# sedaprotocol/bn254

Measured on AMD Instinct MI355X. Metric: BN254 pairings/sec (batch verify), higher is better.
Workload: dtype u32

## Files before the change

### bn254_amd/_native.py

```python
import ctypes
import os
import subprocess

_PKG = os.path.dirname(os.path.abspath(__file__))
_CSRC = os.path.join(_PKG, "csrc")
LIB_PATH = os.environ.get("BN254_LIB", os.path.join(_PKG, "libbn254hip.so"))
import glob


def translation_units():
    return sorted(glob.glob(os.path.join(_CSRC, "*.hip")))


def _dependencies():
    return translation_units() + sorted(glob.glob(os.path.join(_CSRC, "*.h"))) + sorted(glob.glob(os.path.join(_CSRC, "*.inc"))) + [
        os.path.join(_CSRC, "gen_constants.py"), os.path.join(_CSRC, "gen_step_asm.py"), os.path.join(os.path.dirname(_PKG), "include", "bn254_hip.h")]

HIPCC_COMPILE_FLAGS = ["-O3", "--offload-arch=gfx950", "-std=c++17", "-fPIC", "-mllvm", "-amdgpu-sched-strategy=max-ilp"]
HIPCC_LINK_FLAGS = ["--offload-arch=gfx950", "-shared", "-fPIC", "-Wl,--no-undefined"]
HIPCC_FLAGS = HIPCC_COMPILE_FLAGS + ["-shared", "-Wl,--no-undefined"]
_OBJ = os.path.join(_PKG, "build")


def _stale():
# ... 42 lines not shown
            print("libbn254hip.so: %d translation units compiled and linked in %.1f s" % (len(units), time.time() - t0), flush=True)
    return LIB_PATH


_lib = None


def load():
    global _lib
    if _lib is not None:
        return _lib
    if not os.path.exists(LIB_PATH):
        raise RuntimeError("libbn254hip.so is not built (run `python -c 'import __graft_entry__ as g; g.build()'`); "
                           "bn254_amd has no CPU fallback")
    L = ctypes.CDLL(LIB_PATH)
    vp, sz, u32, i32 = ctypes.c_void_p, ctypes.c_size_t, ctypes.c_uint32, ctypes.c_int
    L.bn254_version.restype = ctypes.c_char_p
    L.bn254_ctx_create.argtypes = [i32, ctypes.POINTER(vp)]
    L.bn254_ctx_destroy.argtypes = [vp]
    L.bn254_ctx_destroy.restype = None
    L.bn254_ctx_reserve.argtypes = [vp, sz]
    L.bn254_ctx_reserve_host.argtypes = [vp, sz, sz]
    L.bn254_ctx_synchronize.argtypes = [vp]
    L.bn254_ctx_set_profiling.argtypes = [vp, i32]
    L.bn254_ctx_expect_msgs_len.argtypes = [vp, ctypes.c_uint64]
    L.bn254_ctx_last_kernel_ms.argtypes = [vp, ctypes.POINTER(ctypes.c_float)]
    L.bn254_ctx_set_option.argtypes = [vp, i32, i32]
    L.bn254_debug_route_table.argtypes = [vp, ctypes.POINTER(ctypes.c_uint64), ctypes.POINTER(i32), ctypes.POINTER(i32), i32]
    L.bn254_debug_key_dedup_last.argtypes = [vp, ctypes.POINTER(ctypes.c_uint32)]
    if hasattr(L, "bn254_debug_key_cache_last"):
        L.bn254_debug_key_cache_last.argtypes = [vp, ctypes.POINTER(ctypes.c_uint32)]
    if hasattr(L, "bn254_debug_key_tables"):
        L.bn254_debug_key_tables.argtypes = [vp, i32, sz, sz, vp, vp, vp, vp]
    if hasattr(L, "bn254_debug_agg_tables"):
        L.bn254_debug_agg_tables.argtypes = [vp, i32, sz, sz, vp, vp]
    L.bn254_debug_agg_rand_last.argtypes = [vp, ctypes.POINTER(ctypes.c_uint64)]
    L.bn254_debug_agg_rand_sums.argtypes = [vp, ctypes.POINTER(ctypes.c_uint64), sz, sz, vp, vp, vp, vp, vp, vp]
    L.bn254_ctx_last_clocks.argtypes = [vp, ctypes.POINTER(ctypes.c_double)]
    L.bn254_batch_verify.argtypes = [vp, vp, vp, vp, vp, sz, u32, vp]
    L.bn254_batch_verify_device.argtypes = [vp, vp, vp, vp, vp, sz, u32, vp, vp]
    L.bn254_ctx_register_keys.argtypes = [vp, vp, sz, u32, vp]
    L.bn254_batch_verify_keyed.argtypes = [vp, vp, vp, vp, vp, sz, u32, vp]
    L.bn254_batch_verify_keyed_device.argtypes = [vp, vp, vp, vp, vp, sz, u32, vp, vp]
    L.bn254_batch_verify_keyed_bitmap.argtypes = [vp, vp, vp, vp, vp, sz, sz, u32, vp]
    L.bn254_batch_verify_keyed_bitmap_device.argtypes = [vp, vp, vp, vp, vp, sz, sz, u32, vp, vp]
    L.bn254_batch_verify_keyed_bitmap_randomized.argtypes = [vp, vp, vp, vp, vp, sz, sz, u32, vp, vp]
    L.bn254_batch_verify_keyed_bitmap_randomized_device.argtypes = [vp, vp, vp, vp, vp, sz, sz, u32, vp, vp, vp]
    L.bn254_batch_collect_keyed_bitmap.argtypes = [vp, vp, vp, vp, vp, vp, sz, sz, sz, u32, vp, vp, vp, vp, vp]
    L.bn254_batch_collect_keyed_bitmap_device.argtypes = [vp, vp, vp, vp, vp, vp, sz, sz, sz, u32, vp, vp, vp, vp, vp, vp]
    if hasattr(L, "bn254_batch_collect_keyed_bitmap_randomized"):
        L.bn254_batch_collect_keyed_bitmap_randomized.argtypes = [vp, vp, vp, vp, vp, vp, sz, sz, sz, u32, vp, vp, vp, vp, vp, vp]
        L.bn254_batch_collect_keyed_bitmap_randomized_device.argtypes = [vp, vp, vp, vp, vp, vp, sz, sz, sz, u32, vp, vp, vp, vp, vp, vp, vp]
        L.bn254_debug_collect_rand_last.argtypes = [vp, ctypes.POINTER(ctypes.c_uint64)]
    if hasattr(L, "bn254_batch_collect_keyed_bitmap_optimistic"):
        L.bn254_batch_collect_keyed_bitmap_optimistic.argtypes = [vp, vp, vp, vp, vp, vp, sz, sz, sz, u32, vp, vp, vp, vp, vp]
        L.bn254_batch_collect_keyed_bitmap_optimistic_device.argtypes = [vp, vp, vp, vp, vp, vp, sz, sz, sz, u32, vp, vp, vp, vp, vp, vp]
        L.bn254_debug_collect_opt_last.argtypes = [vp, ctypes.POINTER(ctypes.c_uint64)]
    if hasattr(L, "bn254_batch_merge_keyed_bitmap"):
        L.bn254_batch_merge_keyed_bitmap.argtypes = [vp, vp, vp, vp, vp, vp, sz, sz, sz, u32, vp, vp, vp, vp, vp, vp]
        L.bn254_batch_merge_keyed_bitmap_device.argtypes = [vp, vp, vp, vp, vp, vp, sz, sz, sz, u32, vp, vp, vp, vp, vp, vp, vp]
    L.bn254_debug_bitmap_rand_last.argtypes = [vp, ctypes.POINTER(ctypes.c_uint64)]
    L.bn254_debug_bitmap_rand_sums.argtypes = [vp, ctypes.POINTER(ctypes.c_uint64), sz, sz, vp, vp, vp, vp, vp, vp]
    L.bn254_batch_verify_keyed_randomized.argtypes = [vp, vp, vp, vp, vp, sz, u32, vp, vp]
    L.bn254_batch_verify_keyed_randomized_device.argtypes = [vp, vp, vp, vp, vp, sz, u32, vp, vp, vp]
    L.bn254_batch_verify_compressed.argtypes = [vp, vp, vp, vp, vp, sz, vp]
    L.bn254_batch_verify_compressed_device.argtypes = [vp, vp, vp, vp, vp, sz, vp, vp]
# ... 45 lines not shown
    L.bn254_mgpu_ctx.argtypes = [vp, i32]
    L.bn254_mgpu_ctx.restype = vp
    L.bn254_mgpu_shard_len.argtypes = [vp, sz]
    L.bn254_mgpu_shard_len.restype = sz
    L.bn254_mgpu_gathered_len.argtypes = [vp, sz]
    L.bn254_mgpu_gathered_len.restype = sz
    L.bn254_mgpu_shard_range.argtypes = [vp, sz, i32, ctypes.POINTER(sz), ctypes.POINTER(sz)]
    L.bn254_mgpu_reserve.argtypes = [vp, sz, i32]
    L.bn254_mgpu_synchronize.argtypes = [vp]
    L.bn254_mgpu_set_option.argtypes = [vp, i32, i32]
    L.bn254_mgpu_last_timing.argtypes = [vp, ctypes.POINTER(ctypes.c_float), ctypes.POINTER(ctypes.c_float)]
    L.bn254_mgpu_last_error.argtypes = [vp]
    L.bn254_mgpu_last_error.restype = ctypes.c_char_p
    L.bn254_mgpu_batch_verify.argtypes = [vp, vp, vp, vp, vp, sz, u32, vp]
    L.bn254_mgpu_batch_verify_device.argtypes = [vp, pp, pp, pp, pp, sz, u32, pp, pp]
    L.bn254_mgpu_batch_pairing.argtypes = [vp, vp, vp, sz, sz, u32, vp, vp, ctypes.POINTER(ctypes.c_uint64)]
    L.bn254_mgpu_batch_pairing_device.argtypes = [vp, pp, pp, sz, sz, u32, pp, pp, pp, pp]
    L.bn254_mgpu_batch_hash_to_g1.argtypes = [vp, vp, vp, sz, vp, vp, vp]
    L.bn254_mgpu_batch_verify_compressed.argtypes = [vp, vp, vp, vp, vp, sz, vp]
    L.bn254_mgpu_register_keys.argtypes = [vp, vp, sz, u32, vp]
    L.bn254_mgpu_batch_verify_keyed.argtypes = [vp, vp, vp, vp, vp, sz, u32, vp]
    L.bn254_mgpu_batch_aggregate_verify.argtypes = [vp, vp, vp, sz, vp, sz, vp, vp, vp, vp, sz, u32, vp]
    _lib = L
    return L


EXPORTED_SYMBOLS = [
    "bn254_version", "bn254_ctx_create", "bn254_ctx_destroy", "bn254_ctx_reserve", "bn254_ctx_reserve_host", "bn254_ctx_synchronize",
    "bn254_batch_verify", "bn254_batch_verify_device", "bn254_batch_verify_randomized", "bn254_batch_verify_randomized_device", "bn254_batch_verify_compressed", "bn254_batch_verify_compressed_device", "bn254_batch_hash_to_g1", "bn254_batch_hash_to_g1_device",
    "bn254_batch_pairing_check", "bn254_batch_pairing", "bn254_batch_pairing_device", "bn254_batch_check_public_keys",
    "bn254_batch_g1_add", "bn254_batch_g2_add", "bn254_batch_g1_mul", "bn254_batch_g2_mul", "bn254_batch_g1_mul_device",
    "bn254_batch_g2_mul_device", "bn254_batch_sign", "bn254_batch_sign_device", "bn254_batch_g1_sum", "bn254_batch_g2_sum",
    "bn254_batch_aggregate_verify", "bn254_batch_aggregate_verify_device", "bn254_ctx_register_pools", "bn254_ctx_register_pools_device",
    "bn254_batch_aggregate_verify_registered", "bn254_batch_aggregate_verify_registered_device", "bn254_batch_aggregate_verify_distinct", "bn254_batch_aggregate_verify_distinct_device", "bn254_batch_aggregate_verify_distinct_keyed", "bn254_batch_aggregate_verify_distinct_keyed_device", "bn254_batch_aggregate_verify_distinct_keyed_randomized", "bn254_batch_aggregate_verify_distinct_keyed_randomized_device", "bn254_batch_g1_decompress", "bn254_batch_g2_decompress", "bn254_debug_fp_op", "bn254_debug_fp12_op", "bn254_debug_final_exp_limbs", "bn254_debug_miller_loop", "bn254_debug_hash_candidate", "bn254_debug_route_table", "bn254_debug_key_dedup_last", "bn254_debug_key_cache_last", "bn254_debug_key_tables", "bn254_debug_agg_tables", "bn254_debug_agg_rand_last", "bn254_debug_agg_rand_sums", "bn254_probe_issue_rate", "bn254_probe_leaf_floor", "bn254_probe_fe_program", "bn254_ctx_set_profiling", "bn254_ctx_last_kernel_ms", "bn254_ctx_set_option", "bn254_ctx_last_clocks", "bn254_ctx_expect_msgs_len", "bn254_ctx_register_keys", "bn254_batch_verify_keyed", "bn254_batch_verify_keyed_device", "bn254_batch_verify_keyed_randomized", "bn254_batch_verify_keyed_randomized_device",
    "bn254_batch_verify_keyed_bitmap", "bn254_batch_verify_keyed_bitmap_device",
    "bn254_batch_verify_keyed_bitmap_randomized", "bn254_batch_verify_keyed_bitmap_randomized_device", "bn254_debug_bitmap_rand_last",
    "bn254_debug_bitmap_rand_sums", "bn254_batch_collect_keyed_bitmap", "bn254_batch_collect_keyed_bitmap_device",
    "bn254_batch_collect_keyed_bitmap_randomized", "bn254_batch_collect_keyed_bitmap_randomized_device", "bn254_debug_collect_rand_last",
    "bn254_batch_collect_keyed_bitmap_optimistic", "bn254_batch_collect_keyed_bitmap_optimistic_device", "bn254_debug_collect_opt_last",
    "bn254_batch_merge_keyed_bitmap", "bn254_batch_merge_keyed_bitmap_device",
    "bn254_mgpu_create", "bn254_mgpu_destroy", "bn254_mgpu_device_count", "bn254_mgpu_ctx", "bn254_mgpu_shard_len", "bn254_mgpu_shard_range",
    "bn254_mgpu_gathered_len", "bn254_mgpu_reserve", "bn254_mgpu_synchronize", "bn254_mgpu_set_option", "bn254_mgpu_last_timing",
    "bn254_mgpu_last_error", "bn254_mgpu_batch_verify", "bn254_mgpu_batch_verify_device", "bn254_mgpu_batch_pairing",
    "bn254_mgpu_batch_pairing_device", "bn254_mgpu_batch_hash_to_g1", "bn254_mgpu_batch_verify_compressed", "bn254_mgpu_register_keys",
    "bn254_mgpu_batch_verify_keyed", "bn254_mgpu_batch_aggregate_verify",
]
```

### bn254_amd/csrc/bn254_constants.h

```cpp
#pragma once

#define BN_LIMBS 9
#define BN_W 29
#define BN_MASK 0x1fffffffu
#define BN_HALF 0x10000000
#define BN_QL0 (-126026425)
#define BN_QL1 (17064119)
#define BN_QL2 (-59595953)
#define BN_QL3 (47522513)
#define BN_QL4 (-175777416)
#define BN_QL5 (47923393)
#define BN_QL6 (10936641)
#define BN_QL7 (240920116)
#define BN_QL8 (3171406)
#define BN_QL_ARRAY {BN_QL0, BN_QL1, BN_QL2, BN_QL3, BN_QL4, BN_QL5, BN_QL6, BN_QL7, BN_QL8}
#define BN_N0 0x4866389u
#define BN_TOP_PER_Q 3171406.4
#define BN_R_OVER_Q 169.285
#define BN_WEAK_KMUL 1354
#define BN_WEAK_HALF 1585703
#define BN_U_LO 0x4a6909f1u
#define BN_U_HI 0x44e992b4u
#define BN_N_FIXED_LINES 87

// ... 113 lines not shown
  {{{-200040337, -190665345, 184206374, 76585773, -122040462, 116307427, -3182763, -106971873, 150657}, {-124740882, -48385428, 25363536, -142741679, -158151770, -201941964, -78046412, -104889391, 1502077}}, {{262442771, 34913701, 54788380, -126213246, -261387237, 68871501, -237077543, 122771512, 3009073}, {201181020, -53518767, -160881225, 100319164, 169076449, -54190966, 48482503, 213128087, 857567}}, {{-176370655, -199481511, -128831276, 21759002, 178483129, -45989682, -237679608, 86689705, 903222}, {0, 0, 0, 0, 0, 0, 0, 0, 0}}},
  {{{-199390454, 140322044, -264541497, 218098246, 211463767, 115454738, 123055153, 108741638, 2871680}, {262069691, -87186243, -83201912, 117623600, -30263542, -203954648, 19394695, -190244704, 2253537}}, {{74861434, -57720419, -179314670, -230520040, 65997000, 207431631, 205002456, -66037731, 2120652}, {34392117, -71782572, -264376129, -127196325, 119748025, 203429416, -243176573, -113087350, 1664920}}, {{-176370655, -199481511, -128831276, 21759002, 178483129, -45989682, -237679608, 86689705, 903222}, {0, 0, 0, 0, 0, 0, 0, 0, 0}}},
  {{{-125164594, 203672984, 222121632, -236210239, 29018012, -120395034, -105765485, 146672474, 1819322}, {217134077, -112473868, -13365101, -155118944, 14561761, -163245527, 98054292, -116710799, 1869640}}, {{258779297, 86695130, -41789464, -146609841, -261957730, 146697339, -188270445, 166495143, 27148}, {190558376, -141717460, -92318918, -42801125, 160814942, -243365450, -98538843, 239515481, 2742811}}, {{-176370655, -199481511, -128831276, 21759002, 178483129, -45989682, -237679608, 86689705, 903222}, {0, 0, 0, 0, 0, 0, 0, 0, 0}}},
  {{{-266112787, -5731679, 64851336, 252971724, -4606107, -229625860, -38737421, 232289728, 1646670}, {139400236, -113999012, -78811786, -72939401, 136410247, 92762089, 170592144, 218767022, 1187664}}, {{-148581673, 144737950, -64941939, 266123669, -15806871, -65940181, -120563210, 222667854, 2161520}, {-157986495, 112576346, 175145252, 267211436, -125135784, -183314329, -112175291, -91287041, 2540137}}, {{-176370655, -199481511, -128831276, 21759002, 178483129, -45989682, -237679608, 86689705, 903222}, {0, 0, 0, 0, 0, 0, 0, 0, 0}}},
  {{{179936888, -35473748, -59679566, -5596775, -61480713, 10590727, 16868031, -259608724, 72786}, {176495202, -18815897, -120127598, 178871128, -200921685, 65070547, -58447813, 50527024, 2345596}}, {{208607304, 77283041, -66022222, 42098986, 268119722, 47691154, -142171534, -7679194, 862289}, {124395984, 158373343, -174933619, 134304166, 22689770, 39927471, -178412217, 229699851, 1515716}}, {{-176370655, -199481511, -128831276, 21759002, 178483129, -45989682, -237679608, 86689705, 903222}, {0, 0, 0, 0, 0, 0, 0, 0, 0}}},
  {{{-71531813, 67246960, 237949059, -177971974, -34822371, -224146645, -240850655, -104280605, 2152250}, {-128492592, 30948534, -112506348, 144871973, -7367378, -189697698, -93809008, 62946165, 301481}}, {{159384783, 221847505, -90488723, 22146507, 211531190, 7432841, 132374126, 114003879, 2065160}, {-241377406, 181464060, 7646761, -26472298, -241841179, 120193515, -8498110, -73364135, 1809262}}, {{-176370655, -199481511, -128831276, 21759002, 178483129, -45989682, -237679608, 86689705, 903222}, {0, 0, 0, 0, 0, 0, 0, 0, 0}}},
  {{{-171428400, -249458482, -70035234, 152428224, 268237382, -178271449, 27520838, -120671971, 3068723}, {9932335, -197646614, 142498572, 83337858, -109958741, -179274817, -15833319, -69914058, 96617}}, {{94843765, -103780142, 157119612, -56869585, 15912524, -34614887, 195919263, 64907236, 920143}, {118941173, -98073096, -136818613, 244594129, 129041635, -41694611, 139884983, -259883868, 2705119}}, {{-176370655, -199481511, -128831276, 21759002, 178483129, -45989682, -237679608, 86689705, 903222}, {0, 0, 0, 0, 0, 0, 0, 0, 0}}},
  {{{243121283, -245146285, -156305461, -12818002, -178365131, -177158676, -256937671, 34668348, 75137}, {10333938, -37755957, 72278169, 85086581, 92939512, -72886985, -38751985, -227509480, 925099}}, {{-147192708, 258120271, -41162607, 42078054, -163913536, -119625961, -44844893, 185883765, 1188799}, {235579323, 193778380, -13294417, 159229682, 236601368, 192779425, 13781851, 93907330, 933591}}, {{-176370655, -199481511, -128831276, 21759002, 178483129, -45989682, -237679608, 86689705, 903222}, {0, 0, 0, 0, 0, 0, 0, 0, 0}}},
  {{{-141907892, -107977127, 204683730, 3373323, 96002441, 139722946, -95095458, 134243936, 1812559}, {-185199286, 263934561, 257143555, -179990218, -145893234, -224382509, 102131607, -29198656, 2532873}}, {{-58711793, 245191909, 92638325, 90256483, -67674438, 231377561, -260854161, 176023936, 1608472}, {4908704, -73766975, -173992501, -266421877, -120394349, 39964257, 175000575, 265420786, 33071}}, {{-176370655, -199481511, -128831276, 21759002, 178483129, -45989682, -237679608, 86689705, 903222}, {0, 0, 0, 0, 0, 0, 0, 0, 0}}},
  {{{-214306326, 112995705, 203217010, -45483838, -252784442, 120321467, 186528369, -146789637, 162579}, {-156386064, 217762605, 78321876, 140823106, 185638832, -1785707, -231401731, -203083753, 1261828}}, {{106508173, -117204588, 216647907, 7709844, 200022610, 227507439, 80806348, -181739761, 2784693}, {9540569, -27897884, 155658076, -57119890, -242306310, 11065481, -1829803, -22755391, 2526826}}, {{-176370655, -199481511, -128831276, 21759002, 178483129, -45989682, -237679608, 86689705, 903222}, {0, 0, 0, 0, 0, 0, 0, 0, 0}}},
  {{{-170550275, -131985597, 141986177, 263500420, 33397427, 74369277, 162661307, 152195668, 2661521}, {-81853459, 202864132, 22294944, 1719661, -95127053, -45787432, 169589203, -103112267, 1178675}}, {{-174079808, -51588416, -57795799, 247696906, 234371116, 81952568, 176965714, 50459872, 931029}, {237866458, -125584815, 256714432, 155783857, 144310399, 78795867, 220130107, 123179926, 166919}}, {{-176370655, -199481511, -128831276, 21759002, 178483129, -45989682, -237679608, 86689705, 903222}, {0, 0, 0, 0, 0, 0, 0, 0, 0}}},
  {{{-49306564, -92009915, 76714808, 206425296, -18911896, -89494543, -107789449, 141625555, 1865807}, {234514699, 122766930, -104413407, 106700060, 155636159, 205375446, -46091338, 255081650, 1234052}}, {{-212032201, -36621430, -150832888, -35484420, 162963214, 74033470, -189370026, 17664498, 1423930}, {-163470212, 81285382, -38833882, 108922757, -50181724, -225338663, 149676106, -228450571, 1376109}}, {{-176370655, -199481511, -128831276, 21759002, 178483129, -45989682, -237679608, 86689705, 903222}, {0, 0, 0, 0, 0, 0, 0, 0, 0}}},
  {{{-229545731, -249242282, 48482127, 32812434, -18338362, 126217735, 118954546, 26723153, 3004994}, {-10570593, -188510812, -217780881, -107498616, -165303242, 167964699, -36064246, 75691970, 1723376}}, {{15185324, -47571680, 127749242, -157459636, -41466509, 118054769, -207995470, 153028387, 1037592}, {-39021391, 70955764, 142262821, -130870691, -68729247, -236203824, 80363762, -77152138, 2702413}}, {{-176370655, -199481511, -128831276, 21759002, 178483129, -45989682, -237679608, 86689705, 903222}, {0, 0, 0, 0, 0, 0, 0, 0, 0}}},
  {{{163647724, 192924703, -162630789, -118076012, 142975318, 168169548, -89538170, 62909519, 2094264}, {-214163828, -230767358, -189956325, -157148179, -247498553, -255153517, -236790193, -34715494, 1715569}}, {{115587364, 258688938, -51849393, 78842177, -262068265, -107185610, -221650625, 193176103, 2588549}, {-75559992, 259688436, -77911971, 263346331, 190183004, -143954193, 130301912, -208291216, 317805}}, {{-176370655, -199481511, -128831276, 21759002, 178483129, -45989682, -237679608, 86689705, 903222}, {0, 0, 0, 0, 0, 0, 0, 0, 0}}},
  {{{-21443416, 248752699, 24211503, 180647149, -11004787, -169352692, 24828521, 208236708, 731906}, {240734963, -945267, -94409694, 224890492, -222082203, 95326662, 93146178, -163322462, 3124303}}, {{101170552, 13205284, -256511354, -18535751, -226284632, -14711015, -169989660, 215698512, 1214444}, {-115335139, -243410446, 167591371, 70040109, -111466827, -44550076, 42921127, -61055270, 936229}}, {{-176370655, -199481511, -128831276, 21759002, 178483129, -45989682, -237679608, 86689705, 903222}, {0, 0, 0, 0, 0, 0, 0, 0, 0}}},
  {{{194475413, 66556270, 33163353, 214495719, 84714233, -151129526, 158231720, -178379680, 1711252}, {-23886822, -68860429, -104616143, 50480129, -8681874, 206104951, -153610971, 202107973, 321501}}, {{-265102970, -155790835, 234719479, -118893583, 56555457, 176278835, 16057839, 193352116, 2911462}, {-214060094, -226278758, 210925259, -256654959, -206288843, 143191197, 216026142, -121889172, 2063704}}, {{-176370655, -199481511, -128831276, 21759002, 178483129, -45989682, -237679608, 86689705, 903222}, {0, 0, 0, 0, 0, 0, 0, 0, 0}}},
  {{{211995304, -114933848, -204710941, -153849488, 137386204, -57436494, -268383413, -176836654, 1163802}, {-119692606, -106057472, 24474457, -121620700, -140419497, 254002587, 237930320, 29624771, 1466741}}, {{-33408981, 77861381, -12995667, -26474951, 14983613, -156197272, -230468610, -7322544, 1255074}, {-100843488, 117663684, 224808907, -230128445, -198040350, 198331391, 234252901, 187672035, 1495249}}, {{-176370655, -199481511, -128831276, 21759002, 178483129, -45989682, -237679608, 86689705, 903222}, {0, 0, 0, 0, 0, 0, 0, 0, 0}}},
  {{{258650570, -35612775, -200285181, -53517004, -198078314, 147873122, -124934989, -14800304, 448573}, {198251006, 96238494, -178994434, 246685808, 193583880, -169066857, 132738305, 46917062, 1657838}}, {{-242372727, 175863385, -63652076, 251445205, -120227698, -230194405, -137499659, -69733145, 2549436}, {244579158, -9827117, -175975206, -190679677, -59209720, 68734345, -233140879, -236722399, 958296}}, {{-176370655, -199481511, -128831276, 21759002, 178483129, -45989682, -237679608, 86689705, 903222}, {0, 0, 0, 0, 0, 0, 0, 0, 0}}},
  {{{-118181686, 191380492, 46891918, -67496608, 133499266, 136775164, -30652145, -159719896, 141374}, {111447810, 81254940, 236294220, 176317818, -51431853, 4048663, 76515630, -194841446, 1230674}}, {{-57107160, 30848795, 86177915, 178230363, 173484625, 111107460, -139935602, -160260691, 2613107}, {-14902460, -53830383, -70833480, 265851823, -125813216, -209271761, 172380324, -61621536, 3082156}}, {{-176370655, -199481511, -128831276, 21759002, 178483129, -45989682, -237679608, 86689705, 903222}, {0, 0, 0, 0, 0, 0, 0, 0, 0}}},
  {{{184814613, 51899031, 233603478, 258659516, 153972936, 23890032, -133142987, -88543576, 1729823}, {192270751, -8658243, 214299070, 149087285, 211026243, -164366848, 251037918, -66480647, 1848146}}, {{211883601, 54930164, 101866637, -237060239, -36819856, -9497778, 174962490, 257398535, 482184}, {18982256, -123882900, 239342450, 21201073, -221501387, 220773893, -39037341, -267961371, 1577083}}, {{-176370655, -199481511, -128831276, 21759002, 178483129, -45989682, -237679608, 86689705, 903222}, {0, 0, 0, 0, 0, 0, 0, 0, 0}}},
  {{{-133312880, 263585465, 16353286, 194981750, 46178582, 115018734, -167817870, 139318092, 2068671}, {102282468, 148314672, -30682414, 199717073, -239073256, -242076110, -263081100, 42274790, 1894594}}, {{-105249443, 58595139, 13996760, -101554426, -4112982, 178467927, -44373279, 120348143, 1755967}, {114840994, -148286844, 180095703, -2116349, 92320787, 224277985, 155350517, -133487757, 749870}}, {{-176370655, -199481511, -128831276, 21759002, 178483129, -45989682, -237679608, 86689705, 903222}, {0, 0, 0, 0, 0, 0, 0, 0, 0}}},
  {{{-48534465, -216407913, -80449945, 197826411, 28844792, -79138690, -244010556, 186112668, 655732}, {-135627737, -219576662, -43600977, 162482618, 166965224, -181199647, 124866808, 75750459, 1878572}}, {{-74728592, -13595521, -87696240, -51211358, 144286912, 201058004, 12627411, -252447748, 2293052}, {31278092, -87291687, 250215026, 250101657, -122853210, 185162931, 115541449, -237945290, 2101663}}, {{-176370655, -199481511, -128831276, 21759002, 178483129, -45989682, -237679608, 86689705, 903222}, {0, 0, 0, 0, 0, 0, 0, 0, 0}}},
  {{{1920732, -177274209, -94106247, -259622463, 198105170, -77279384, 152108594, 207918834, 273777}, {-137525945, 121461598, -13360930, 249712992, 198210032, 30308474, -77309931, -199784788, 734443}}, {{263023313, -259909195, -178730994, -171277393, -50243763, -207558859, 132438671, -254036575, 2614219}, {2299910, -80464943, 249430672, 178951382, 4286762, 184744822, 154232506, 259713016, 120390}}, {{-176370655, -199481511, -128831276, 21759002, 178483129, -45989682, -237679608, 86689705, 903222}, {0, 0, 0, 0, 0, 0, 0, 0, 0}}},
  {{{-166807573, 257561474, 5758311, 16562045, 154704719, -115989712, 30296549, 212095792, 2382072}, {-214218106, 109893984, 260431646, 253247344, 185804414, 147228457, -149769418, -248037657, 2745144}}, {{254155362, -31231806, -262802243, 127284760, 189343100, -188982993, 50947556, 54876934, 753175}, {-181976431, -56200449, -228230263, 261245934, -133178743, 254970581, 132113466, -232840218, 2676942}}, {{-176370655, -199481511, -128831276, 21759002, 178483129, -45989682, -237679608, 86689705, 903222}, {0, 0, 0, 0, 0, 0, 0, 0, 0}}},
  {{{37112481, 129068714, 2231463, 118245711, 73714168, 14136474, -227005073, 114158147, 1452017}, {-241524548, -219338631, -195709013, -49076846, -61142324, 95780292, -127092311, -233650515, 105673}}, {{42977708, -76007726, 195561301, -171725564, -264048364, 121600305, -211248172, 30495361, 460408}, {216640771, -129426574, -148041264, -106105658, 8450471, 125953370, -107989583, 70858773, 2231587}}, {{-176370655, -199481511, -128831276, 21759002, 178483129, -45989682, -237679608, 86689705, 903222}, {0, 0, 0, 0, 0, 0, 0, 0, 0}}},
  {{{-3232440, -230912943, -165435285, -161296496, 181300732, -186576993, 158514743, -102527308, 178806}, {213156407, -97026260, 105562298, -60297714, -35770377, -231575633, 106944355, 130250462, 2063018}}, {{-265998852, 226199746, 182911214, -64753753, 196257397, -115603873, 257355951, -248162796, 1250972}, {-43343060, -31181880, -185052752, 87259796, -169372165, -102536487, 194779497, -263472281, 973169}}, {{-176370655, -199481511, -128831276, 21759002, 178483129, -45989682, -237679608, 86689705, 903222}, {0, 0, 0, 0, 0, 0, 0, 0, 0}}},
  {{{88056784, -7863797, 2393509, 189566777, -4124281, 43222830, 74388923, 115793747, 1596681}, {-61490741, 166590202, -262009048, -241222290, 151032788, 152243465, -198708223, 133601828, 1001776}}, {{170428225, 28120576, 158580597, -267158179, -205070664, -193272982, -118866539, 48154750, 763669}, {-87919621, 83255079, -89948094, 44678235, 224783456, 153742904, 120397335, -139364349, 1815208}}, {{-176370655, -199481511, -128831276, 21759002, 178483129, -45989682, -237679608, 86689705, 903222}, {0, 0, 0, 0, 0, 0, 0, 0, 0}}},
  {{{262805377, 25131819, -207131569, -169166008, -77129595, -74240946, -108282114, -244472810, 517945}, {-93130162, -94355081, 64587666, 84777866, -90920406, -8820760, 139744111, 142454513, 1344638}}, {{84178301, -101967244, -185592134, 124907746, 8864191, -181416434, 175900991, 37214613, 2250176}, {-71996750, -249770878, 32060657, 100694729, -248824792, 157385725, -54255296, -114993530, 1691525}}, {{-176370655, -199481511, -128831276, 21759002, 178483129, -45989682, -237679608, 86689705, 903222}, {0, 0, 0, 0, 0, 0, 0, 0, 0}}},
  {{{4468045, -257270474, -212501869, -201875648, 247931930, -69039740, -10866934, -159837900, 418727}, {-195131113, -26854457, -113740685, -179567795, 87499462, -64426147, -249940327, 257223239, 2328593}}, {{127008600, 119343077, 52409536, -7940586, 111211957, 54407389, -42873706, 203151225, 3108489}, {231539509, -140691144, -164724047, -33026607, 26982684, -156904521, 265339498, -46944075, 2243270}}, {{-176370655, -199481511, -128831276, 21759002, 178483129, -45989682, -237679608, 86689705, 903222}, {0, 0, 0, 0, 0, 0, 0, 0, 0}}},
  {{{-44891955, 90630318, -67087730, 24812910, 95403380, 185541070, 22421094, -48123712, 1870376}, {-114359724, 212759385, -155669803, -13087971, 118129017, -193674558, -98888558, 197073061, 793579}}, {{89208724, -233383300, -79197354, -1132594, -265691887, 247209455, -245705599, -187369324, 99477}, {206283919, -105467383, -216114661, 73440443, -137125806, -220635920, -73680286, 25048480, 941390}}, {{-176370655, -199481511, -128831276, 21759002, 178483129, -45989682, -237679608, 86689705, 903222}, {0, 0, 0, 0, 0, 0, 0, 0, 0}}},
  {{{-162397500, 2954997, 152488182, -65669248, -2226221, 126434462, 136504248, -45920178, 1018187}, {37038594, -230220348, -39757353, 51278743, 94503435, 69559177, 117383119, -38335104, 1747986}}, {{-168849216, 266245294, 103631925, -116049438, -183139901, -68554844, 259384813, -968803, 1609363}, {215323032, -48099119, -244987994, -57467655, -73007447, -145862608, -75994125, -187878897, 359235}}, {{-176370655, -199481511, -128831276, 21759002, 178483129, -45989682, -237679608, 86689705, 903222}, {0, 0, 0, 0, 0, 0, 0, 0, 0}}},
  {{{198924502, -95920802, 109010388, 97989720, -212428967, 216061620, -144460110, 93801757, 1223757}, {-249735650, 57427941, 134749786, -254932027, 35573088, 90419683, 133149999, 143547148, 125881}}, {{194882581, 87312206, -43835174, -161184211, 204737166, -171525322, -265395304, 139734743, 2318771}, {-210600565, -38893026, 17554950, -242192057, 58146045, -142126381, 157173323, 44273995, 2017346}}, {{-176370655, -199481511, -128831276, 21759002, 178483129, -45989682, -237679608, 86689705, 903222}, {0, 0, 0, 0, 0, 0, 0, 0, 0}}},
};
```

### bn254_amd/csrc/bn254_devhooks.hip

```cpp
#include <hip/hip_runtime.h>

#include <cstdio>
#include <cstdlib>
#include <cstring>
#include <new>

#include "../../include/bn254_hip.h"
#include "bn254_hash.h"
#include "bn254_io.h"
#include "bn254_pairing.h"

using namespace bn254;

#include "bn254_ws.h"
#include "bn254_lane.h"
#include "bn254_host.h"

KERNEL_SMALL void k_debug_fp_op(int op, const uint8_t* a, const uint8_t* b, size_t n, uint8_t* out, uint8_t* status) {
  size_t i = (size_t)blockIdx.x * BN_WAVE + threadIdx.x;
  if (i >= n) return;
  uint32_t any = 0;
  Fp x, y, r;
  bool ok = fp_from_be(x, a + 32 * i, any);
  if (b) ok = fp_from_be(y, b + 32 * i, any) && ok; else y = fp_zero();
// ... 192 lines not shown
    if (!c->kd_last_run || !c->kd_ctl || !c->kd_lines_last) return BN254_E_BAD_ARGUMENT;
    HIP_TRY(hipMemcpy(ctl, c->kd_ctl, sizeof ctl, hipMemcpyDeviceToHost));
    if (first + count > ctl[KD_CTL_D] || first + count > c->kd_keys_cap) return BN254_E_BAD_ARGUMENT;
    if (ctl[KD_CTL_BUILD] + ctl[KD_CTL_HITS] != ctl[KD_CTL_D]) return BN254_E_BAD_ARGUMENT;
    if (rep) HIP_TRY(hipMemcpy(rep, c->kd_rep_last + first, count * sizeof(uint32_t), hipMemcpyDeviceToHost));
    const size_t cap = c->kd_keys_cap;
    uint8_t* h = (uint8_t*)malloc(count * sizeof(uint32_t) + 2 * cap + 1);
    if (!h) return BN254_E_NO_MEMORY;
    const uint32_t* rows = (const uint32_t*)h;
    uint8_t *h_st = h + count * sizeof(uint32_t), *h_inf = h_st + cap;
    hipError_t e = count ? hipMemcpy(h, c->kd_row_of_last + first, count * sizeof(uint32_t), hipMemcpyDeviceToHost) : hipSuccess;
    if (e == hipSuccess) e = hipMemcpy(h_st, c->kd_st_last, cap, hipMemcpyDeviceToHost);
    if (e == hipSuccess) e = hipMemcpy(h_inf, c->kd_inf_last, cap, hipMemcpyDeviceToHost);
    int rc = e == hipSuccess ? 0 : -(int)e;
    for (size_t k = 0; k < count && !rc; ++k) {
      const size_t r = rows[k];
      if (r >= cap) { rc = BN254_E_BAD_ARGUMENT; break; }
      e = hipMemcpy(lines + k * per_key, c->kd_lines_last + r * per_key, per_key * sizeof(int32_t), hipMemcpyDeviceToHost);
      if (e != hipSuccess) rc = -(int)e;
      if (st) st[k] = h_st[r];
      if (inf) inf[k] = h_inf[r];
    }
    free(h);
    return rc;
  } else {
    if (!c->key_lines || first + count > c->n_keys) return BN254_E_BAD_ARGUMENT;
    src = c->key_lines; src_st = c->key_st; src_inf = c->key_inf;
  }
  HIP_TRY(hipMemcpy(lines, src + first * per_key, count * per_key * sizeof(int32_t), hipMemcpyDeviceToHost));
  if (st) HIP_TRY(hipMemcpy(st, src_st + first, count, hipMemcpyDeviceToHost));
  if (inf) HIP_TRY(hipMemcpy(inf, src_inf + first, count, hipMemcpyDeviceToHost));
  return 0;
}
static int debug_rand_last(bn254_ctx* c, int ran, const uint32_t* stats, uint64_t out[6]) {
  if (!c || !out) return BN254_E_BAD_ARGUMENT;
  for (int i = 0; i < 6; ++i) out[i] = 0;
  if (!ran || !stats) return 0;
  HIP_TRY(hipSetDevice(c->device));
  HIP_TRY(hipDeviceSynchronize());
  uint32_t st[5];
  HIP_TRY(hipMemcpy(st, stats, sizeof st, hipMemcpyDeviceToHost));
  out[0] = 1;
  for (int i = 0; i < 5; ++i) out[i + 1] = st[i];
  return 0;
}
int bn254_debug_agg_rand_last(bn254_ctx* c, uint64_t out[6]) { return debug_rand_last(c, c ? c->aggr_last_ran : 0, c ? c->aggr_stats : nullptr, out); }
int bn254_debug_bitmap_rand_last(bn254_ctx* c, uint64_t out[6]) { return debug_rand_last(c, c ? c->bmr_last_ran : 0, c ? c->bmr_stats : nullptr, out); }
int bn254_debug_collect_rand_last(bn254_ctx* c, uint64_t out[4]) {
  if (!c || !out) return BN254_E_BAD_ARGUMENT;
  for (int i = 0; i < 4; ++i) out[i] = 0;
  if (!c->clr_last_ran || !c->clr_stats) return 0;
  HIP_TRY(hipSetDevice(c->device));
  HIP_TRY(hipDeviceSynchronize());
  uint32_t st[4];
  HIP_TRY(hipMemcpy(st, c->clr_stats, sizeof st, hipMemcpyDeviceToHost));
  for (int i = 0; i < 4; ++i) out[i] = st[i];
  return 0;
}
int bn254_debug_collect_opt_last(bn254_ctx* c, uint64_t out[4]) {
  if (!c || !out) return BN254_E_BAD_ARGUMENT;
  for (int i = 0; i < 4; ++i) out[i] = 0;
  if (!c->clo_last_ran || !c->clo_stats) return 0;
  HIP_TRY(hipSetDevice(c->device));
  HIP_TRY(hipDeviceSynchronize());
  uint32_t st[4];
  HIP_TRY(hipMemcpy(st, c->clo_stats, sizeof st, hipMemcpyDeviceToHost));
// ... 206 lines not shown
```

### bn254_amd/csrc/bn254_hip.hip

```cpp
#include <hip/hip_runtime.h>
#include <thread>

#include <cstdio>
#include <cstdlib>
#include <cstring>
#include <new>

#include "../../include/bn254_hip.h"
#include "bn254_hash.h"
#include "bn254_io.h"
#include "bn254_pairing.h"

using namespace bn254;

#include "bn254_ws.h"
#include "bn254_lane.h"
#include "bn254_host.h"

KERNEL_SMALL void k_decode_g1(const uint8_t* pts, size_t n, uint32_t flags, Ws ws, int px, int inf_plane, int accumulate) {
  size_t i = (size_t)blockIdx.x * BN_WAVE + threadIdx.x;
  if (i >= n) return;
  G1Affine p;
  uint8_t st = decode_g1(p, pts + 64 * i, flags);
  if (st != ST_OK) g1_set_generator(p);
// ... 392 lines not shown
  if (c->max_chunk > 0) return n > (size_t)c->max_chunk ? (size_t)c->max_chunk : 0;
  if (n * ws_per_item <= c->ws.stride && (!key_dedup || (n <= c->kd_items_cap && (size_t)c->kd_max_keys <= c->kd_keys_cap))) return 0;
  const size_t per_item = ws_per_item * WS_BYTES_PER_ITEM + (key_dedup ? KD_BYTES_PER_ITEM : 0);
  const size_t fixed = key_dedup ? (size_t)c->kd_max_keys * KD_BYTES_PER_KEY : 0;
  size_t avail;
  if (c->assume_free_mb > 0) avail = (size_t)c->assume_free_mb << 20;
  else {
    size_t fr = 0, total = 0;
    if (hipSetDevice(c->device) != hipSuccess || hipMemGetInfo(&fr, &total) != hipSuccess) { (void)hipGetLastError(); return 0; }
    avail = fr + c->ws.stride * WS_BYTES_PER_ITEM + c->kd_items_cap * KD_BYTES_PER_ITEM + c->kd_keys_cap * KD_BYTES_PER_KEY;
  }
  const size_t need = ((n + 255) & ~(size_t)255) * per_item + fixed;
  if (need <= avail / 10 * 9) return 0;
  const size_t room = avail / 10 * 8 > fixed ? avail / 10 * 8 - fixed : 0;
  size_t chunk = room / per_item;
  chunk &= ~(size_t)65535;
  if (chunk == 0) chunk = room / per_item & ~(size_t)255;
  if (key_dedup && (chunk == 0 || route_for(c, chunk).miller != BN_ML_LANE_PAIRS)) return ws_chunk_for(c, n, ws_per_item, false);
  return chunk && chunk < n ? chunk : 0;
}
#define KD_NO_ROOM 1
static int kd_reserve(bn254_ctx* c, size_t n, KeyDedup& kd) {
  size_t slots = 1;
  while (slots < 2 * n) slots <<= 1;
  const size_t keys = (size_t)c->kd_max_keys;
  if (n > c->kd_items_cap || keys > c->kd_keys_cap) {
    const size_t items_cap = n > c->kd_items_cap ? ((n + 255) & ~(size_t)255) : c->kd_items_cap;
    const size_t keys_cap = keys > c->kd_keys_cap ? keys : c->kd_keys_cap;
    { int rc_ = ctx_quiesce(c); if (rc_) return rc_; }
    if (c->kd_buf) { HIP_TRY(hipFree(c->kd_buf)); c->kd_buf = nullptr; }
    c->kd_items_cap = c->kd_keys_cap = 0;
    c->kd_ctl = nullptr;
    c->kd_lines_last = nullptr;
    c->kd_cache_valid = false;
    if (hipMalloc((void**)&c->kd_buf, items_cap * KD_BYTES_PER_ITEM + keys_cap * KD_BYTES_PER_KEY + 512) != hipSuccess) {
      (void)hipGetLastError();
      c->kd_buf = nullptr;
      return KD_NO_ROOM;
    }
    c->kd_items_cap = items_cap;
    c->kd_keys_cap = keys_cap;
  }
  size_t slots_cap = 1;
  while (slots_cap < 2 * c->kd_items_cap) slots_cap <<= 1;
  uint8_t* p = c->kd_buf;
  auto take = [&](size_t bytes) { uint8_t* r = p; p += (bytes + 15) & ~(size_t)15; return r; };
  kd.table = (uint32_t*)take(slots_cap * 4);
  kd.slot_id = (uint32_t*)take(slots_cap * 4);
  kd.slot_of = (uint32_t*)take(c->kd_items_cap * 4);
  kd.key_idx = (uint32_t*)take(c->kd_items_cap * 4);
  kd.lines = (int32_t*)take(c->kd_keys_cap * BN_N_FIXED_LINES * BN_KEY_LINE_WORDS * 4);
  kd.c2 = (int32_t*)take(c->kd_keys_cap * BN_N_FIXED_LINES * 2 * BN_LIMBS * 4);
  kd.rep = (uint32_t*)take(c->kd_keys_cap * 4);
  kd.ctl = (uint32_t*)take(KD_CTL_WORDS * 4);
  c->kd_ctl = kd.ctl;
  kd.st = take(c->kd_keys_cap);
  kd.inf = take(c->kd_keys_cap);
  kd.row_of = (uint32_t*)take(c->kd_keys_cap * 4);
  kd.build_row = (uint32_t*)take(c->kd_keys_cap * 4);
  kd.build_rep = (uint32_t*)take(c->kd_keys_cap * 4);
  kd.c_keys = (uint32_t*)take(c->kd_keys_cap * 128);
  size_t index_slots = 1;
  while (index_slots < 2 * keys) index_slots <<= 1;
  kd.c_index = (uint32_t*)take(4 * c->kd_keys_cap * 4);
  kd.c_state = (uint32_t*)take(4);
  kd.index_mask = (uint32_t)(index_slots - 1);
  c->kd_lines_last = kd.lines; c->kd_rep_last = kd.rep; c->kd_st_last = kd.st; c->kd_inf_last = kd.inf; c->kd_row_of_last = kd.row_of;
  kd.slot_mask = (uint32_t)(slots - 1);
  kd.hash_mask = c->kd_hash_bits > 0 && c->kd_hash_bits < 32 ? (1u << c->kd_hash_bits) - 1 : 0xFFFFFFFFu;
  kd.max_keys = (uint32_t)keys;
  kd.min_mult = (uint32_t)c->kd_min_mult;
  return 0;
}
int scratch_reserve(bn254_ctx* c, uint8_t** buf, size_t* cap, size_t bytes) {
  if (bytes <= *cap) return 0;
  { int rc_ = ctx_quiesce(c); if (rc_) return rc_; }
  if (*buf) { HIP_TRY(hipFree(*buf)); *buf = nullptr; *cap = 0; }
  const size_t grown = (bytes + 4095) & ~(size_t)4095;
  HIP_TRY(hipMalloc((void**)buf, grown));
  *cap = grown;
  return 0;
}
int stage_reserve(bn254_ctx* c, int slot, size_t bytes) {
  if (bytes <= c->stage_cap[slot]) return 0;
  HIP_TRY(hipSetDevice(c->device));
  return scratch_reserve(c, &c->stage[slot], &c->stage_cap[slot], bytes);
}
uint8_t* HostStaging::out(int slot, size_t bytes, void* host) {
  if (!rc) rc = stage_reserve(c, slot, bytes);
  if (rc) return nullptr;
  if (host) copy_back(host, c->stage[slot], bytes);
  return c->stage[slot];
}
uint8_t* HostStaging::in(int slot, const void* host, size_t bytes) {
  uint8_t* d = out(slot, bytes ? bytes : 1);
  if (d && bytes) check(hipMemcpyAsync(d, host, bytes, hipMemcpyHostToDevice, c->stream));
  return rc ? nullptr : d;
}
void HostStaging::copy_back(void* host, const void* dev, size_t bytes) {
  if (!host || !bytes) return;
// ... 170 lines not shown
  c->pair_lanes = 1;
  c->rand_min_batch = RAND_MIN_BATCH_DEFAULT;
  c->agg_rand_min_pairs = AGG_RAND_MIN_PAIRS_DEFAULT;
  c->agg_rand_group_pairs = AGG_RAND_GROUP_PAIRS_DEFAULT;
  c->bmr_min_tuples = BITMAP_RAND_MIN_TUPLES_DEFAULT;
  c->bmr_group_tuples = BITMAP_RAND_GROUP_TUPLES_DEFAULT;
  c->bmr_max_keys = BITMAP_RAND_MAX_KEYS_DEFAULT;
  c->collect_wave_min = COLLECT_WAVE_MIN_SHARES_DEFAULT;
  c->collect_rand_min_shares = COLLECT_RAND_MIN_SHARES_DEFAULT;
  c->collect_rand_min_per_key = COLLECT_RAND_MIN_PER_KEY_DEFAULT;
  c->collect_opt_min_shares = COLLECT_OPT_MIN_SHARES_DEFAULT;
  c->collect_opt_min_tuple_shares = COLLECT_OPT_MIN_TUPLE_SHARES_DEFAULT;
  c->merge_wave_min = MERGE_WAVE_MIN_PARTS_DEFAULT;
  c->trio_max_batch = TRIO_MAX_BATCH_DEFAULT;
  c->hash_direct_width = HASH_DIRECT_WIDTH_DEFAULT;
  c->hash_tail_chunk = HASH_TAIL_CHUNK_DEFAULT;
  c->trio_wave_roles = TRIO_WAVE_ROLES_DEFAULT;
  c->agg_subset_min_tuples = AGG_SUBSET_MIN_TUPLES_DEFAULT;
  c->agg_sort_by_msg = 1;
  c->agg_t4_route = 0;
  c->agg_wide_min_tuples = AGG_WIDE_MIN_TUPLES_DEFAULT;
  c->pinned_staging = PINNED_STAGING_DEFAULT;
  c->fits_w8 = bn254_quad_fits_device(1); c->fits_quad = bn254_quad_fits_device(0); c->fits_trio = bn254_trio_fits_device();
  if (c->trio_wave_roles == 2 && !c->fits_w8) c->trio_wave_roles = 1;
  if (c->trio_wave_roles == 1 && !c->fits_quad) c->trio_wave_roles = 0;
  if (!c->fits_trio) c->trio_max_batch = 0;
  c->nonet_max_batch = bn254_nonet_fits_device() ? NONET_MAX_BATCH_DEFAULT : 0;
  c->lm_max_batch = bn254_lm_fits_device() ? LM_MAX_BATCH_DEFAULT : 0;
  c->nonet_wide = 1;
  c->g2_fixed_base = 1;
  c->key_dedup = 1;
  c->kd_max_keys = KEY_DEDUP_MAX_KEYS_DEFAULT;
  c->kd_min_mult = KEY_DEDUP_MIN_MULT_DEFAULT;
  c->kd_cache = 1;
  c->bm_table_max_keys = BITMAP_TABLE_MAX_KEYS_DEFAULT;
  c->device = hip_device;
  hipError_t err = hipStreamCreateWithFlags(&c->stream, hipStreamNonBlocking);
  if (err == hipSuccess) err = hipStreamCreateWithFlags(&c->copy_stream, hipStreamNonBlocking);
  if (err == hipSuccess) err = hipEventCreateWithFlags(&c->copy_done, hipEventDisableTiming);
  if (err == hipSuccess) err = hipEventCreateWithFlags(&c->last_done, hipEventDisableTiming);
  if (err == hipSuccess) err = hipStreamCreateWithFlags(&c->kd_stream, hipStreamNonBlocking);
  if (err == hipSuccess) err = hipEventCreateWithFlags(&c->kd_fork, hipEventDisableTiming);
  if (err == hipSuccess) err = hipEventCreateWithFlags(&c->kd_join, hipEventDisableTiming);
  if (err == hipSuccess) err = hipEventCreateWithFlags(&c->kd_done, hipEventDisableTiming);
  for (int i = 0; i < 5 && err == hipSuccess; ++i) err = hipEventCreate(&c->ev[i]);
  if (err != hipSuccess) {
    if (c->kd_done) (void)hipEventDestroy(c->kd_done);
    if (c->kd_join) (void)hipEventDestroy(c->kd_join);
    if (c->kd_fork) (void)hipEventDestroy(c->kd_fork);
    if (c->kd_stream) (void)hipStreamDestroy(c->kd_stream);
    if (c->last_done) (void)hipEventDestroy(c->last_done);
    for (int i = 0; i < 5; ++i) if (c->ev[i]) (void)hipEventDestroy(c->ev[i]);
    if (c->copy_done) (void)hipEventDestroy(c->copy_done);
    if (c->copy_stream) (void)hipStreamDestroy(c->copy_stream);
    if (c->stream) (void)hipStreamDestroy(c->stream);
    delete c;
    return -(int)err;
  }
  *out = c;
  return 0;
}
void bn254_ctx_destroy(bn254_ctx* c) {
  if (!c) return;
  (void)hipSetDevice(c->device);
  (void)ctx_quiesce(c);
  if (c->ws.planes) (void)hipFree(c->ws.planes);
// ... 94 lines not shown
    c->nonet_max_batch = value;
    return 0;
  }
  if (option == BN254_OPT_NONET_WIDE) { c->nonet_wide = value != 0; return 0; }
  if (option == BN254_OPT_LM_MAX_BATCH) {
    HIP_TRY(hipSetDevice(c->device));
    if (value < 0 || (value > 0 && !bn254_lm_fits_device())) return BN254_E_BAD_ARGUMENT;
    c->lm_max_batch = value;
    return 0;
  }
  if (option == BN254_OPT_PINNED_STAGING) { if (value < 0 || value > 16) return BN254_E_BAD_ARGUMENT; c->pinned_staging = value; return 0; }
  if (option == BN254_OPT_AGG_SORT_BY_MSG) { c->agg_sort_by_msg = value != 0; return 0; }
  if (option == BN254_OPT_AGG_T4_ROUTE) { if (value < 0 || value > 1) return BN254_E_BAD_ARGUMENT; c->agg_t4_route = value; return 0; }
  if (option == BN254_OPT_AGG_WIDE_MIN_TUPLES) { if (value < 0) return BN254_E_BAD_ARGUMENT; c->agg_wide_min_tuples = value; return 0; }
  if (option == BN254_OPT_CLOCK_PROBE) {
    HIP_TRY(hipSetDevice(c->device));
    HIP_TRY(hipDeviceSynchronize());
    if (value && !c->ws.clk) {
      HIP_TRY(hipMalloc((void**)&c->ws.clk, sizeof(unsigned long long) * 3 * BN_CLK_MAX_WG * 2));
      HIP_TRY(hipMemset(c->ws.clk, 0, sizeof(unsigned long long) * 3 * BN_CLK_MAX_WG * 2));
    } else if (!value && c->ws.clk) {
      HIP_TRY(hipFree(c->ws.clk));
      c->ws.clk = nullptr;
    }
    return 0;
  }
  if (option == BN254_OPT_HASH_MAX_TRIES) { if (value < 0 || value > 255) return BN254_E_BAD_ARGUMENT; c->hash_max_tries = value; return 0; }
  if (option == BN254_OPT_G2_FIXED_BASE) { c->g2_fixed_base = value != 0; return 0; }
  if (option == BN254_OPT_MAX_CHUNK) { if (value < 0) return BN254_E_BAD_ARGUMENT; c->max_chunk = value; return 0; }
  if (option == BN254_OPT_ASSUME_FREE_MB) { if (value < 0) return BN254_E_BAD_ARGUMENT; c->assume_free_mb = value; return 0; }
  if (option == BN254_OPT_KEY_DEDUP) { if (value < 0 || value > 1) return BN254_E_BAD_ARGUMENT; c->key_dedup = value; return 0; }
  if (option == BN254_OPT_KEY_DEDUP_MAX_KEYS) { if (value < 0 || value > KEY_DEDUP_MAX_KEYS_LIMIT) return BN254_E_BAD_ARGUMENT; c->kd_max_keys = value; return 0; }
  if (option == BN254_OPT_KEY_DEDUP_MIN_MULT) { if (value < 1) return BN254_E_BAD_ARGUMENT; c->kd_min_mult = value; return 0; }
  if (option == BN254_OPT_KEY_DEDUP_FORCE_GENERIC) { c->kd_force_generic = value == 2 ? 2 : value != 0; return 0; }
  if (option == BN254_OPT_KEY_CACHE) { if (value < 0 || value > 1) return BN254_E_BAD_ARGUMENT; c->kd_cache = value; c->kd_cache_valid = false; return 0; }
  if (option == BN254_OPT_KEY_DEDUP_HASH_BITS) { if (value < 0 || value > 32) return BN254_E_BAD_ARGUMENT; c->kd_hash_bits = value; return 0; }
  if (option == BN254_OPT_AGGD_KEYED_ROUTE) { if (value < 0 || value > 3) return BN254_E_BAD_ARGUMENT; c->aggd_keyed_route = value; return 0; }
  if (option == BN254_OPT_AGG_RAND_MIN_PAIRS) { if (value < 0) return BN254_E_BAD_ARGUMENT; c->agg_rand_min_pairs = value; return 0; }
  if (option == BN254_OPT_AGG_RAND_GROUP_PAIRS) { if (value < 1) return BN254_E_BAD_ARGUMENT; c->agg_rand_group_pairs = value; return 0; }
  if (option == BN254_OPT_BITMAP_TABLE_MAX_KEYS) { if (value < 0) return BN254_E_BAD_ARGUMENT; c->bm_table_max_keys = value; return 0; }
  if (option == BN254_OPT_BITMAP_RAND_MIN_TUPLES) { if (value < 0) return BN254_E_BAD_ARGUMENT; c->bmr_min_tuples = value; return 0; }
  if (option == BN254_OPT_BITMAP_RAND_MAX_KEYS) { if (value < 0) return BN254_E_BAD_ARGUMENT; c->bmr_max_keys = value; return 0; }
  if (option == BN254_OPT_COLLECT_WAVE_MIN_SHARES) { if (value < 1) return BN254_E_BAD_ARGUMENT; c->collect_wave_min = value; return 0; }
  if (option == BN254_OPT_COLLECT_RAND_MIN_SHARES) { if (value < 0) return BN254_E_BAD_ARGUMENT; c->collect_rand_min_shares = value; return 0; }
  if (option == BN254_OPT_COLLECT_RAND_MIN_PER_KEY) { if (value < 0) return BN254_E_BAD_ARGUMENT; c->collect_rand_min_per_key = value; return 0; }
  if (option == BN254_OPT_COLLECT_OPT_MIN_SHARES) { if (value < 0) return BN254_E_BAD_ARGUMENT; c->collect_opt_min_shares = value; return 0; }
  if (option == BN254_OPT_MERGE_WAVE_MIN_PARTS) { if (value < 1) return BN254_E_BAD_ARGUMENT; c->merge_wave_min = value; return 0; }
  if (option == BN254_OPT_COLLECT_OPT_MIN_TUPLE_SHARES) { if (value < 0) return BN254_E_BAD_ARGUMENT; c->collect_opt_min_tuple_shares = value; return 0; }
  if (option == BN254_OPT_BITMAP_RAND_GROUP_TUPLES) { if (value < 1) return BN254_E_BAD_ARGUMENT; c->bmr_group_tuples = value; return 0; }
  if (option == BN254_OPT_BITMAP_ROUTE) { if (value < 0 || value > 2) return BN254_E_BAD_ARGUMENT; c->bm_route = value; return 0; }
  return BN254_E_BAD_ARGUMENT;
}
int bn254_ctx_last_clocks(bn254_ctx* c, double sclk_mhz[3]) {
  if (!c || !sclk_mhz || !c->ws.clk) return BN254_E_BAD_ARGUMENT;
  HIP_TRY(hipSetDevice(c->device));
  int wall_khz = 0;
  HIP_TRY(hipDeviceGetAttribute(&wall_khz, hipDeviceAttributeWallClockRate, c->device));
  const size_t words = (size_t)3 * BN_CLK_MAX_WG * 2;
  unsigned long long* h = (unsigned long long*)malloc(words * sizeof(unsigned long long));
  if (!h) return BN254_E_NO_MEMORY;
  hipError_t e = hipDeviceSynchronize();
  if (e == hipSuccess) e = hipMemcpy(h, c->ws.clk, words * sizeof(unsigned long long), hipMemcpyDeviceToHost);
  if (e == hipSuccess) e = hipMemset(c->ws.clk, 0, words * sizeof(unsigned long long));
  if (e != hipSuccess) { free(h); return -(int)e; }
  for (int k = 0; k < 3; ++k) {
    double cyc = 0, wall = 0;
// ... 30 lines not shown
    default: return bn254_pair_final_exp(n, c->ws, use_hash, d_status, nullptr, nullptr, s);
  }
}
int launch_verify_miller_fe(bn254_ctx* c, hipStream_t s, size_t n, int pairs, int use_hash, uint8_t* d_status, bool mark) {
  if (!c->pair_lanes) {
    const unsigned g = grid_for(n);
    if (pairs == BN_PAIRS_CHECK_PKS) k_miller_cpk<<<g, BN_WAVE, 0, s>>>(n, c->ws);
    else k_miller_verify<<<g, BN_WAVE, 0, s>>>(n, c->ws, nullptr, nullptr);
    if (mark) PROF_MARK(3);
    k_final_exp<<<g, BN_WAVE, 0, s>>>(n, 1, 1, 1, c->ws, use_hash, nullptr, d_status, 0, 0, nullptr, nullptr);
    return 0;
  }
  const BnRoute r = route_for(c, n);
  int rc;
  switch (r.miller) {
    case BN_ML_LANE_MACHINE: rc = bn254_lm_miller_verify(n, c->ws, s, pairs); break;
    case BN_ML_WAVE_ROLES:
      rc = c->trio_wave_roles == 2 ? bn254_w8_miller_verify(n, c->ws, s, pairs)
           : c->trio_wave_roles ? bn254_quad_miller_verify(n, c->ws, s, pairs) : bn254_trio_miller_verify(n, c->ws, s, pairs);
      break;
    default: rc = bn254_pair_miller_verify(n, c->ws, nullptr, nullptr, s, pairs); break;
  }
  if (rc) return rc;
  if (mark) PROF_MARK(3);
  return launch_final_exp_layout(c, s, n, use_hash, d_status, r.fe);
}

extern "C" {
static int verify_tail(bn254_ctx* c, hipStream_t s, size_t n, uint8_t* d_status, bool split, const KeyDedup* kd, int hash_first) {
  int rc;
  if (kd) {
    HIP_TRY(hipStreamWaitEvent(s, c->kd_join, 0));
    const KeyTable kt = {kd->lines, kd->st, kd->inf, kd->max_keys};
    if ((rc = bn254_pair_miller_verify_keyed(n, c->ws, kd->key_idx, kt, s, 0, nullptr, kd->ctl + KD_CTL_KEYED_N))) return rc;
    if ((rc = bn254_pair_miller_verify(n, c->ws, nullptr, kd->ctl + KD_CTL_GENERIC_N, s))) return rc;
    PROF_MARK(3);
    if ((rc = bn254_pair_final_exp(n, c->ws, 1, d_status, nullptr, nullptr, s))) return rc;
    HIP_TRY(hipEventRecord(c->kd_done, s));
  } else if (split) {
    const unsigned g = grid_for(n);
    k_miller_verify_split<<<2 * g, BN_WAVE, 0, s>>>(n, c->ws.stride / 2, g, c->ws);
    PROF_MARK(3);
    k_final_exp<<<g, BN_WAVE, 0, s>>>(n, 2, 1, c->ws.stride / 2, c->ws, 1, nullptr, d_status, 0, 0, nullptr, nullptr);
  } else if ((rc = launch_verify_miller_fe(c, s, n, BN_PAIRS_VERIFY, 1, d_status, true))) return rc;
  PROF_MARK(4);
  prof_done(c, hash_first ? EV_HASH_FIRST : EV_DECODE_FIRST);
  HIP_TRY(hipGetLastError());
  return 0;
}
static int verify_after_decode(bn254_ctx* c, hipStream_t s, const uint8_t* d_msgs, const uint64_t* d_off, size_t n, uint8_t* d_status, bool split,
                               const KeyDedup* kd = nullptr) {
  PROF_MARK(1);
  if (const int rc = launch_hash_rounds(c, s, d_msgs, d_off, n, PL_P2X, BY_P2_INF, nullptr)) return rc;
  PROF_MARK(2);
  return verify_tail(c, s, n, d_status, split, kd, 0);
}

int bn254_batch_verify_device(bn254_ctx* c, const uint8_t* d_msgs, const uint64_t* d_off, const uint8_t* d_sigs, const uint8_t* d_pks,
                              size_t n, uint32_t flags, uint8_t* d_status, void* stream) {
  MsgsLenScope msgs_len_scope(c);
  if (!c || (n && (!d_msgs || !d_off || !d_sigs || !d_pks || !d_status))) return BN254_E_BAD_ARGUMENT;
  if (n == 0) return 0;
  if (misaligned(d_sigs) || misaligned(d_pks) || ((uintptr_t)d_off & 7u)) return BN254_E_MISALIGNED;
  HIP_TRY(hipSetDevice(c->device));
  bool split = c->split_miller && n <= BN_SPLIT_MAX_N;
  bool key_dedup = c->key_dedup && c->kd_max_keys > 0 && c->pair_lanes && !split && n <= 0xFFFFFFFFu &&
                         route_for(c, n).miller == BN_ML_LANE_PAIRS && route_for(c, n).fe == BN_FE_LANE_PAIRS;
// ... 309 lines not shown
```

### bn254_amd/csrc/bn254_host.h

```cpp
#pragma once
#include <hip/hip_runtime.h>

#include <cstdint>
#include <cstdlib>
#include <cstring>
#include <new>

#include "../../include/bn254_hip.h"

#define BN_HIDDEN __attribute__((visibility("hidden")))

struct AggTables { int valid; size_t n_msgs, n_signers, n_groups, groups4, built_for; int wide2, wide1, t4_builder; };

struct AggrLast { size_t ng, cbase, tbase; const uint32_t *nagg, *bkey; const uint64_t *glo, *ghi; const uint8_t* gst; };

enum EvLayout { EV_DECODE_FIRST = 0, EV_HASH_FIRST = 1, EV_COLLECT = 2 };

struct bn254_ctx {
  int device;
  hipStream_t stream;
  Ws ws;
  uint8_t* stage[8];
  size_t stage_cap[8];
  int profiling;
// ... 21 lines not shown
  int ev_valid;
  int ev_layout;
  hipStream_t copy_stream;
  uint8_t* pin;
  size_t pin_cap;
  int pinned_staging;
  hipEvent_t copy_done;
  uint64_t msgs_len_next;
  int msgs_len_declared;
  uint64_t msgs_len_call;
  int entry_depth;
  int32_t* key_lines;
  int32_t* key_xy;
  uint8_t* key_st;
  uint8_t* key_inf;
  size_t n_keys, key_cap;
  hipEvent_t last_done;
  bool last_done_armed;
  Pool g2_comb;
  int g2_comb_ready;
  Pool g1_comb;
  int g1_comb_ready;
  int g2_fixed_base;
  AggTables reg_pools;
  int max_chunk;
  int assume_free_mb;
  bool fits_w8, fits_quad, fits_trio;
  uint8_t* aggd_buf;
  size_t aggd_cap;
  int key_dedup;
  int kd_max_keys;
  int kd_min_mult;
  int kd_force_generic;
  int kd_hash_bits;
  hipStream_t kd_stream;
  hipEvent_t kd_fork, kd_join;
  hipEvent_t kd_done;
  int kd_cache;
  bool kd_cache_valid;
  uint32_t kd_cache_flags;
  int kd_cache_max_keys, kd_cache_hash_bits;
  uint8_t* kd_buf;
  size_t kd_items_cap, kd_keys_cap;
  uint32_t* kd_ctl;
  const int32_t* kd_lines_last;
  const uint32_t* kd_rep_last;
  const uint32_t* kd_row_of_last;
  const uint8_t *kd_st_last, *kd_inf_last;
  int kd_last_run;
  int aggd_keyed_route;
  int agg_rand_min_pairs;
  int agg_rand_group_pairs;
  uint8_t* aggr_buf;
  size_t aggr_cap;
  uint32_t* aggr_stats;
  int aggr_last_ran;
  AggrLast aggr_last;
  uint8_t* bm_bad;
  size_t bm_bad_cap;
  uint8_t* bm_tab;
  size_t bm_tab_cap;
  bool bm_bad_valid, bm_tab_valid;
  int bm_table_max_keys;
  int bm_route;
  int bmr_min_tuples;
  int bmr_group_tuples;
  int bmr_max_keys;
  uint8_t* bmr_buf;
  size_t bmr_cap;
  uint32_t* bmr_stats;
  int bmr_last_ran;
  AggrLast bmr_last;
  uint8_t* collect_buf;
  size_t collect_cap;
  int collect_wave_min;
  int collect_rand_min_shares;
  int collect_rand_min_per_key;
  uint32_t* clr_stats;
// ... 150 lines not shown
```

### bn254_amd/csrc/bn254_keydedup.h

```cpp
#pragma once

namespace bn254 {

template <class Emit>
BN_DEV bool kd_walk_raw_lines(const G2Affine& q, Emit&& emit) {
  G2Proj t;
  LineCoef l;
  t.x = q.x; t.y = q.y; t.z = fp2_one();
  const Fp2 q_yneg = fp2_neg(q.y);
  bool degenerate = false;
  int idx = 0;
  auto line = [&]() {
    const Fp2 c2 = NR(290, l.c2);
    degenerate = fp2_is_zero(c2) || degenerate;
    emit(idx++, NS(292, l.c0), NS(293, l.c1), c2);
  };
#if defined(__HIPCC__)
#pragma clang loop unroll(disable)
#endif
  for (int d = 0; d < 64; ++d) {
    dbl_step(t, l); line();
    const int digit = C_ATE_NAF[d];
    if (digit != 0) { add_step(t, l, q.x, fp2_select(digit > 0, q.y, q_yneg)); line(); }
  }
  add_step(t, l, fp2_mul(fp2_conj(q.x), fp2_load_const(C_TW_FROB_X1)), fp2_mul(fp2_conj(q.y), fp2_load_const(C_TW_FROB_Y1))); line();
  add_step(t, l, fp2_mul(q.x, fp2_load_const(C_TW_FROB_X2)), q.y); line();
  return degenerate;
}
BN_DEV void kd_scale_line(const Fp2& c0, const Fp2& c1, const Fp2& c2, Fp2& r0, Fp2& r1) {
  const Fp2 inv = NS(291, fp2_inv(c2));
  const Fp2 a = fp2_mul(c0, inv), b = fp2_mul(c1, inv);
  BN_FOR_ROLES(k) { r0.c[k] = fp_canon(a.c[k]); r1.c[k] = fp_canon(b.c[k]); }
}

#define KD_TREE_LEAVES 128
#define KD_TREE_LEVELS 7
#if !defined(__HIPCC__)
static inline void kd_scale_tree(const Fp2* c0, const Fp2* c1, const Fp2* c2, Fp2* r0, Fp2* r1) {
  static_assert(BN_N_FIXED_LINES <= KD_TREE_LEAVES && (1 << KD_TREE_LEVELS) == KD_TREE_LEAVES, "tree shape");
  Fp2 prod[2 * KD_TREE_LEAVES], inv[2 * KD_TREE_LEAVES];
  for (int p = 0; p < KD_TREE_LEAVES; ++p) prod[KD_TREE_LEAVES + p] = p < BN_N_FIXED_LINES ? fp2_reduce_weak(c2[p]) : fp2_one();
  for (int w = KD_TREE_LEAVES / 2; w >= 1; w >>= 1)
    for (int node = w; node < 2 * w; ++node) prod[node] = fp2_mul(prod[2 * node], prod[2 * node + 1]);
  inv[1] = fp2_inv(prod[1]);
  for (int w = 2; w <= KD_TREE_LEAVES; w <<= 1)
    for (int node = w; node < 2 * w; ++node) inv[node] = fp2_mul(inv[node >> 1], prod[node ^ 1]);
  for (int p = 0; p < BN_N_FIXED_LINES; ++p) {
    const Fp2 a = fp2_mul(c0[p], inv[KD_TREE_LEAVES + p]), b = fp2_mul(c1[p], inv[KD_TREE_LEAVES + p]);
    BN_FOR_ROLES(k) { r0[p].c[k] = fp_canon(a.c[k]); r1[p].c[k] = fp_canon(b.c[k]); }
  }
}
#endif

#if defined(__HIPCC__)
BN_DEV bool load_fp_be_checked(Fp& r, const uint8_t* p, uint32_t& any) {
  const uint32_t* w = (const uint32_t*)p;
  U256 t;
#pragma unroll
  for (int k = 0; k < 8; ++k) { t.w[7 - k] = __builtin_bswap32(w[k]); any |= w[k]; }
  bool ok = !u256_geq(t.w, C_Q);
  r = fp_from_u256(t);
  return ok;
}
BN_DEV uint8_t decode_g2_pair_role(G2Affine& q, const uint8_t* b, uint32_t flags) {
  const unsigned role = threadIdx.x & 1u;
  uint32_t any = 0;
  bool ok = load_fp_be_checked(q.x.c[0], b + 32 * role, any);
  ok = load_fp_be_checked(q.y.c[0], b + 64 + 32 * role, any) && ok;
  any |= (uint32_t)bn_partner_word((int32_t)any);
  ok = bn_pair_and(ok);
  q.inf = any == 0;
  uint8_t st = ST_OK;
  if (q.inf) st = (flags & FLAG_REJECT_IDENTITY) ? (uint8_t)ST_INVALID_GROUP_POINT : (uint8_t)ST_OK;
  else if (!ok) st = ST_NOT_MEMBER;
  const bool on_curve = g2_on_curve(q);
  if (st == ST_OK && !q.inf && !on_curve) st = ST_INVALID_GROUP_POINT;
  return st;
}
#endif

}
```

### bn254_amd/csrc/bn254_keydedup.hip

```cpp
#include <hip/hip_runtime.h>

#define BN_SPLIT_FP2 1
#define bn254 bn254_kd
#include "bn254_pairing.h"
#include "bn254_keydedup.h"
#include "bn254_lmachine.h"
#include "bn254_kdlines.h"

using namespace bn254;

#include "bn254_ws.h"

#define KD_WG 256
#define KERNEL_KD_PAIR __global__ __launch_bounds__(KD_WG) __attribute__((amdgpu_waves_per_eu(2, 2)))
#define KERNEL_KD __global__ __launch_bounds__(KD_WG)

__device__ __forceinline__ uint32_t kd_hash(const uint32_t* w, uint32_t hash_mask) {
  uint32_t h = 0x9E3779B9u;
#pragma unroll
  for (int k = 0; k < 32; ++k) {
    h ^= w[k];
    h *= 0x85EBCA6Bu;
    h ^= h >> 13;
  }
// ... 185 lines not shown
    if (live && pair < 3) kd_store_own(c == 2 ? c2s + (size_t)idx * 2 * BN_LIMBS : rows + (size_t)idx * BN_KEY_LINE_WORDS + (size_t)c * 2 * BN_LIMBS, v);
  }
};
KERNEL_KD_LM void k_kd_lines(const uint8_t* pks, uint32_t flags, KeyDedup kd, int report_degenerate) {
  const uint32_t d = kd.ctl[KD_CTL_BUILD];
  if ((uint32_t)blockIdx.x * KD_LM_PER_WAVE >= d) return;
  __builtin_amdgcn_s_setprio(3);
  const unsigned l = threadIdx.x, v = l / KD_LM_LANES, role = l & 1u;
  KdLmDev m;
  m.writer = v < KD_LM_PER_WAVE;
  const unsigned vslot = m.writer ? v : KD_LM_PER_WAVE - 1;
  m.pair = (l % KD_LM_LANES) >> 1;
  uint32_t j = (uint32_t)blockIdx.x * KD_LM_PER_WAVE + vslot;
  m.live = m.writer && j < d;
  if (j >= d) j = d - 1;
  const uint32_t row = kd.build_row[j];
  m.bx.base = vslot * KD_LM_KEY_STRIDE + role * KD_LM_ROLE_STRIDE;
  G2Affine q;
  const uint8_t st = decode_g2_pair_role(q, pks + 128 * (size_t)kd.build_rep[j], flags);
  const bool real = st == ST_OK && !q.inf;
  if (!real) { q.x = fp2_load_const(C_G2_GEN[0]); q.y = fp2_load_const(C_G2_GEN[1]); }
  if (m.live && m.pair == 0 && role == 0) { kd.st[row] = st; kd.inf[row] = q.inf; }
  if (m.writer) {
    m.bx.put(m.bx.slot(LS_ZERO), fp2_zero()); m.bx.put(m.bx.slot(LS_DUMMY), fp2_zero());
    kd_builder_init(m.bx, q);
  }
#pragma unroll
  for (int lv = 0; lv < KD_LV_N; ++lv) {
    const LmEntry* t = kd_level_table(lv);
#pragma unroll
    for (int k = 0; k < 5; ++k) m.e[lv].w[k] = t[m.pair].w[k];
  }
  m.rows = kd.lines + (size_t)row * BN_N_FIXED_LINES * BN_KEY_LINE_WORDS;
  m.c2s = kd.c2 + (size_t)row * BN_N_FIXED_LINES * 2 * BN_LIMBS;
  m.degenerate = false;
  KD_LM_FENCE();
  kd_builder_program(m);
  if (m.live && ((real && m.degenerate) || report_degenerate) && m.pair == 0 && role == 0) atomicOr(&kd.ctl[KD_CTL_FLAGS], (uint32_t)KD_DEGENERATE);
}
static_assert(BN_N_FIXED_LINES <= KD_TREE_LEAVES && 2 * KD_TREE_LEAVES == KD_WG, "one lane pair per leaf");
#define KD_NODE_WORDS (2 * BN_LIMBS)
KERNEL_KD_PAIR void k_kd_scale(KeyDedup kd) {
  if (blockIdx.x >= kd.ctl[KD_CTL_BUILD]) return;
  const uint32_t j = kd.build_row[blockIdx.x];
  __shared__ int32_t prod[2 * KD_TREE_LEAVES * KD_NODE_WORDS];
  __shared__ int32_t inv[2 * KD_TREE_LEAVES * KD_NODE_WORDS];
  const uint32_t p = threadIdx.x >> 1;
  const bool line = p < BN_N_FIXED_LINES;
  int32_t* row = kd.lines + ((size_t)j * BN_N_FIXED_LINES + (line ? p : 0u)) * BN_KEY_LINE_WORDS;
  {
    Fp2 leaf = fp2_one();
    if (line) leaf = fp2_reduce_weak(kd_load_own(kd.c2 + ((size_t)j * BN_N_FIXED_LINES + p) * KD_NODE_WORDS));
    kd_store_own(prod + (KD_TREE_LEAVES + p) * KD_NODE_WORDS, leaf);
  }
  __syncthreads();
  for (uint32_t w = KD_TREE_LEAVES / 2; w >= 1; w >>= 1) {
    if (p < w) {
      const uint32_t node = w + p;
      kd_store_own(prod + node * KD_NODE_WORDS, fp2_mul(kd_load_own(prod + 2 * node * KD_NODE_WORDS), kd_load_own(prod + (2 * node + 1) * KD_NODE_WORDS)));
    }
    __syncthreads();
  }
  if (threadIdx.x < BN_WAVE) {
    const Fp2 r = fp2_inv(kd_load_own(prod + KD_NODE_WORDS));
    if (p == 0) kd_store_own(inv + KD_NODE_WORDS, r);
  }
  __syncthreads();
  for (uint32_t w = 2; w <= KD_TREE_LEAVES; w <<= 1) {
    if (p < w) {
      const uint32_t node = w + p;
      kd_store_own(inv + node * KD_NODE_WORDS, fp2_mul(kd_load_own(inv + (node >> 1) * KD_NODE_WORDS), kd_load_own(prod + (node ^ 1u) * KD_NODE_WORDS)));
    }
    __syncthreads();
  }
  if (!line) return;
  const Fp2 c2inv = kd_load_own(inv + (KD_TREE_LEAVES + p) * KD_NODE_WORDS);
  const Fp2 a = fp2_mul(kd_load_own(row), c2inv), b = fp2_mul(kd_load_own(row + 2 * BN_LIMBS), c2inv);
  Fp2 r0, r1;
  BN_FOR_ROLES(k) { r0.c[k] = fp_canon(a.c[k]); r1.c[k] = fp_canon(b.c[k]); }
  kd_store_own(row, r0);
  kd_store_own(row + 2 * BN_LIMBS, r1);
}
KERNEL_KD void k_kd_decide(size_t n, KeyDedup kd, int force_generic, int cache_on) {
  const bool keyed = force_generic != 1 && kd_viable(kd, n) && (kd.ctl[KD_CTL_FLAGS] & KD_DEGENERATE) == 0;
  if (threadIdx.x == 0) {
    kd.ctl[KD_CTL_KEYED_N] = keyed ? (uint32_t)n : 0u;
    kd.ctl[KD_CTL_GENERIC_N] = keyed ? 0u : (uint32_t)n;
  }
  if (!keyed || !cache_on) return;
  const uint32_t built = kd.ctl[KD_CTL_BUILD];
  for (uint32_t m = threadIdx.x; m < built; m += KD_WG) {
    const uint32_t row = kd.build_row[m];
    uint32_t w[32];
#pragma unroll
    for (int k = 0; k < 32; ++k) w[k] = kd.c_keys[(size_t)row * 32 + k];
    const uint32_t h = kd_hash(w, kd.hash_mask);
    for (uint32_t probe = 0; probe <= kd.index_mask; ++probe)
      if (atomicCAS(&kd.c_index[(h + probe) & kd.index_mask], KD_EMPTY, row) == KD_EMPTY) break;
  }
  if (threadIdx.x == 0) kd.c_state[0] += built;
}

int bn254_kd_enqueue(const uint8_t* d_pks, size_t n, uint32_t flags, KeyDedup kd, int force_generic, int cache_reset, int cache_on, hipStream_t s) {
  HIP_TRY(hipMemsetAsync(kd.table, 0xFF, ((size_t)kd.slot_mask + 1) * sizeof(uint32_t), s));
  HIP_TRY(hipMemsetAsync(kd.ctl, 0, KD_CTL_WORDS * sizeof(uint32_t), s));
  const unsigned g = (unsigned)((n + KD_WG - 1) / KD_WG);
  k_kd_insert<<<g, KD_WG, 0, s>>>(d_pks, n, kd);
  k_kd_match<<<1, KD_MATCH_WG, 0, s>>>(d_pks, n, kd, cache_reset || !cache_on);
  k_kd_resolve<<<g, KD_WG, 0, s>>>(n, kd);
  k_kd_lines<<<(unsigned)((kd.max_keys + KD_LM_PER_WAVE - 1) / KD_LM_PER_WAVE), BN_WAVE, KD_LM_LDS_WORDS * sizeof(int32_t), s>>>(d_pks, flags, kd, force_generic == 2);
  k_kd_scale<<<kd.max_keys, KD_WG, 0, s>>>(kd);
  k_kd_decide<<<1, KD_WG, 0, s>>>(n, kd, force_generic, cache_on);
  HIP_TRY(hipGetLastError());
  return 0;
// ... 2 lines not shown
```

### bn254_amd/csrc/bn254_pair.hip

```cpp
#include <hip/hip_runtime.h>

#define BN_SPLIT_FP2 1
#if defined(BN_PAIR_FP6_LAZY) && !defined(BN_FP6_LAZY)
#define BN_FP6_LAZY 1
#endif
#ifndef BN_PAIR_NO_SQR_DPP_ASM
#define BN_PAIR_SQR_DPP_ASM 1
#endif
#ifndef BN_PAIR_CALL_FP12_HOT
#define BN_INLINE_FP12_HOT 1
#endif
#ifndef BN_PAIR_CALL_MUL_LINE
#define BN_INLINE_MUL_LINE 1
#endif
#ifndef BN_PAIR_CALL_FE_HOT
#define BN_INLINE_FE_HOT 1
#endif
#ifndef BN_PRIO_SHIFT
#define BN_PRIO_SHIFT 1
#endif
#define BN_SET_STEP_PRIORITY(step)                                                        \
  do {                                                                                    \
    if (((step) & ((1 << BN_PRIO_SHIFT) - 1)) == 0) {                                     \
      int q_ = ((step) >> BN_PRIO_SHIFT) & 3;                                             \
// ... 124 lines not shown
  BN_CLK_END(ws, 0);
  ws_store_f12_own(ws, i, f);
}
KERNEL_PAIR void k_miller_verify_keyed_pair(size_t n, Ws ws, const uint32_t* key_idx, KeyTable kt, size_t base, const uint32_t* map,
                                            const uint32_t* count) {
  size_t i = ((size_t)blockIdx.x * BN_PAIR_WG + threadIdx.x) >> 1;
  if (i >= n) return;
  if (count && i >= *count) return;
  if (map) i = map[i];
  uint32_t key = key_idx[i];
  i += base;
  uint8_t kst = ST_OK;
  if (key >= kt.n_keys) { kst = ST_INDEX_OOB; key = 0; }
  else kst = kt.st[key];
  const bool key_inf = kst != ST_OK || kt.inf[key] != 0;
  if ((threadIdx.x & 1u) == 0) {
    const uint8_t prev = ws_byte(ws, BY_ST_DECODE, i);
    ws_byte(ws, BY_ST_DECODE, i) = prev != ST_OK ? prev : kst;
  }
  G1Affine sig, h;
  ws_load_g1(ws, PL_P1X, BY_P1_INF, i, sig);
  ws_load_g1(ws, PL_P2X, BY_P2_INF, i, h);
  __shared__ Fp12PairSlot lds_f[BN_PAIR_WG];
  Fp12& f = lds_f[threadIdx.x].v;
  typedef const int32_t (*LinePtr)[2][2][BN_LIMBS];
  BN_CLK_BEGIN(ws);
  miller_loop_keyed<true>(f, h, key_inf, (LinePtr)(kt.lines + (size_t)key * BN_N_FIXED_LINES * BN_KEY_LINE_WORDS), sig);
  BN_CLK_END(ws, 0);
  ws_store_f12_own(ws, i, f);
}
int bn254_pair_miller_verify_keyed(size_t n, Ws ws, const uint32_t* key_idx, KeyTable kt, hipStream_t s, size_t base, const uint32_t* map,
                                   const uint32_t* count) {
  k_miller_verify_keyed_pair<<<(unsigned)((2 * n + BN_PAIR_WG - 1) / BN_PAIR_WG), BN_PAIR_WG, 0, s>>>(n, ws, key_idx, kt, base, map, count);
  HIP_TRY(hipGetLastError());
  return 0;
}
KERNEL_PAIR void k_miller_var_pair(size_t n, Ws ws) {
  size_t i = ((size_t)blockIdx.x * BN_PAIR_WG + threadIdx.x) >> 1;
  if (i >= n) return;
  G1Affine p;
  G2Affine q;
  ws_load_g1(ws, PL_P1X, BY_P1_INF, i, p);
  q.x = ws_load_fp2_own(ws, PL_QX0, i);
  q.y = ws_load_fp2_own(ws, PL_QY0, i);
  q.inf = ws_byte(ws, BY_Q_INF, i) != 0;
  __shared__ Fp12PairSlot lds_f[BN_PAIR_WG];
  Fp12& f = lds_f[threadIdx.x].v;
  miller_loop<true, false, true>(f, p, q, p);
  ws_store_f12_own(ws, i, f);
}
template <int ITEMS_PER_PAIR>
__device__ __forceinline__ void miller_rand_pair_body(size_t n, size_t n_groups, Ws ws, size_t gbase) {
  constexpr unsigned PAIRS_PER_GROUP = BN_WAVE / ITEMS_PER_PAIR;
  constexpr unsigned GROUPS_PER_WG = (BN_PAIR_WG / 2) / PAIRS_PER_GROUP;
  const unsigned pair = threadIdx.x >> 1, gp = pair / PAIRS_PER_GROUP, tp = pair % PAIRS_PER_GROUP;
  const size_t group = (size_t)blockIdx.x * GROUPS_PER_WG + gp;
  const size_t i0 = group * BN_WAVE + (size_t)tp * ITEMS_PER_PAIR;
  __shared__ Fp12PairSlot lds_f[BN_PAIR_WG];
  Fp12& f = lds_f[threadIdx.x].v;
  G1Affine a0;
  G2Affine pk0;
  const size_t j0 = i0 < n ? i0 : n - 1;
  ws_load_g1(ws, PL_HASHX, BY_A_INF, j0, a0);
  if (i0 >= n) a0.inf = true;
  pk0.x = ws_load_fp2_own(ws, PL_QX0, j0); pk0.y = ws_load_fp2_own(ws, PL_QY0, j0); pk0.inf = ws_byte(ws, BY_Q_INF, j0) != 0;
  if constexpr (ITEMS_PER_PAIR == 2) {
// ... 541 lines not shown
```

### bn254_amd/csrc/bn254_pairing.h

```cpp
#pragma once
#include "bn254_curve.h"


namespace bn254 {

struct G2Proj { Fp2 x, y, z; };
struct LineCoef { Fp2 c0, c1, c2; };

BN_DEVN void dbl_step(G2Proj& t, LineCoef& l) {
  Fp2 xy = fp2_mul(t.x, t.y), b = fp2_sqr(t.y), c = fp2_sqr(t.z);
  Fp2 e = fp2_mul(c, fp2_load_const(C_TWIST_3B));
  Fp2 f = fp2_add(fp2_dbl(e), e);
  Fp2 h = fp2_sub(fp2_sub(fp2_sqr(NS(200, fp2_add(t.y, t.z))), b), c);
  Fp2 x2 = fp2_sqr(t.x);
  Fp2 e2x4 = NS(201, fp2_dbl(fp2_dbl(fp2_sqr(e))));
  Fp2 e2x12 = fp2_add(fp2_dbl(e2x4), e2x4);
  G2Proj o;
  o.x = NS(203, fp2_mul(fp2_dbl(xy), NS(202, fp2_sub(b, f))));
  o.y = NS(205, fp2_sub(fp2_sqr(NS(204, fp2_add(b, f))), e2x12));
  o.z = NS(206, fp2_dbl(fp2_dbl(fp2_mul(b, h))));
  l.c0 = h;
  l.c1 = fp2_neg(fp2_add(fp2_dbl(x2), x2));
  l.c2 = fp2_sub(b, e);
  t = o;
// ... 146 lines not shown
    b0.c1 = fp2_select(skip_a || skip_b, zero, b0.c1);
    b0.c2 = fp2_select(skip_a || skip_b, zero, b0.c2);
    b10 = fp2_select(both, zero, fp2_select(only_a, m1, fp2_select(only_b, l1, b10)));
    b11 = fp2_select(both, zero, fp2_select(skip_a || skip_b, one, b11));
  }
  fp12_mul_line2(f, f, b0, b10, b11);
}
template <bool F_LDS = false>
BN_DEVM void miller_loop_keyed(Fp12& f, const G1Affine& pa, bool key_inf, const int32_t (*tab)[2][2][BN_LIMBS], const G1Affine& pb) {
  if constexpr (F_LDS) BN_ASSUME_LDS(&f);
  fp12_set_one(f);
  const bool skip_a = pa.inf || key_inf, skip_b = pb.inf;
#if defined(__HIPCC__)
  const bool any_skip = __builtin_amdgcn_ballot_w64(skip_a || skip_b) != 0;
#else
  const bool any_skip = skip_a || skip_b;
#endif
  int idx = 0;
  auto step = [&]() {
    KeyLine la;
    la.c0 = fp2_load_const(tab[idx][0]); la.c1 = fp2_load_const(tab[idx][1]);
    mul_by_two_table_lines(f, la, pa.x, pa.y, skip_a, idx, pb.x, pb.y, skip_b, any_skip);
    ++idx;
  };
  for (int d = 0; d < 64; ++d) {
    BN_SET_STEP_PRIORITY(d);
    fp12_sqr(f, f);
    step();
    if (C_ATE_NAF[d] != 0) step();
  }
  step();
  step();
}
BN_DEV void mul_by_two_key_lines(Fp12& f, const KeyLine& la, const Fp& pax, const Fp& pay, bool skip_a, const KeyLine& lb, const Fp& pbx, const Fp& pby,
                                 bool skip_b, bool any_skip) {
  const Fp2 l0 = fp2_mul_fp(la.c0, pay), l1 = fp2_mul_fp(la.c1, pax);
  const Fp2 m0 = fp2_mul_fp(lb.c0, pby), m1 = fp2_mul_fp(lb.c1, pbx);
  const Fp2 v0 = fp2_mul(l0, m0), v1 = fp2_mul(l1, m1);
  const Fp2 x01 = fp2_sub(fp2_sub(fp2_mul(NS(280, fp2_add(l0, l1)), NS(281, fp2_add(m0, m1))), v0), v1);
  Fp6 b0;
  b0.c0 = NS(282, fp2_add(v0, fp2_load_const(C_XI_MONT))); b0.c1 = v1; b0.c2 = NS(283, fp2_add(l1, m1));
  Fp2 b10 = NS(284, x01), b11 = NS(285, fp2_add(l0, m0));
  if (any_skip) {
    const Fp2 one = fp2_one(), zero = fp2_zero();
    const bool both = skip_a && skip_b, only_a = skip_a && !skip_b, only_b = skip_b && !skip_a;
    b0.c0 = fp2_select(both, one, fp2_select(only_a, m0, fp2_select(only_b, l0, b0.c0)));
    b0.c1 = fp2_select(skip_a || skip_b, zero, b0.c1);
    b0.c2 = fp2_select(skip_a || skip_b, zero, b0.c2);
    b10 = fp2_select(both, zero, fp2_select(only_a, m1, fp2_select(only_b, l1, b10)));
    b11 = fp2_select(both, zero, fp2_select(skip_a || skip_b, one, b11));
  }
  fp12_mul_line2(f, f, b0, b10, b11);
}
template <int W, bool F_LDS = false>
BN_DEVM void miller_loop_tables(Fp12& f, const G1Affine& pa, bool skip_a, const int32_t (*taba)[2][2][BN_LIMBS], const G1Affine& pb, bool skip_b,
                                const int32_t (*tabb)[2][2][BN_LIMBS]) {
  static_assert(W == 1 || W == 2, "one or two table pairs per lane pair");
  if constexpr (F_LDS) BN_ASSUME_LDS(&f);
  fp12_set_one(f);
#if defined(__HIPCC__)
  const bool any_skip = __builtin_amdgcn_ballot_w64(skip_a || (W == 2 && skip_b)) != 0;
#else
  const bool any_skip = skip_a || (W == 2 && skip_b);
#endif
  int idx = 0;
  auto step = [&]() {
// ... 770 lines not shown
```

### bn254_amd/csrc/bn254_ws.h

```cpp
#pragma once
#include <stddef.h>

#define BN_WAVE 64
#define BN_SPLIT_MAX_N ((size_t)98304)
#define TRIO_MAX_BATCH_DEFAULT 16384
#define NONET_WIDE_MAX_BATCH 1024
#define NONET_MAX_BATCH_DEFAULT 3072
#define LM_MAX_BATCH_DEFAULT 1536
enum BnMillerLayout { BN_ML_LANE_MACHINE = 0, BN_ML_WAVE_ROLES = 1, BN_ML_LANE_PAIRS = 2 };
enum BnFeLayout { BN_FE_NONET_WIDE = 0, BN_FE_NONET = 1, BN_FE_OCTET = 2, BN_FE_LANE_PAIRS = 3 };
struct BnRouteLimits { size_t lm_max, nonet_wide_max, nonet_max, small_max; };
struct BnRoute { int miller, fe; };
static inline BnRoute bn_route(const BnRouteLimits& L, size_t n) {
  BnRoute r = {BN_ML_LANE_PAIRS, BN_FE_LANE_PAIRS};
  if (n > L.small_max) return r;
  r.miller = n <= L.lm_max ? BN_ML_LANE_MACHINE : BN_ML_WAVE_ROLES;
  r.fe = n <= L.nonet_max ? (n <= L.nonet_wide_max ? BN_FE_NONET_WIDE : BN_FE_NONET) : BN_FE_OCTET;
  return r;
}
static inline int bn_route_table(const BnRouteLimits& L, size_t* max_n, BnRoute* route, int cap) {
  size_t b[4] = {L.lm_max, L.nonet_wide_max, L.nonet_max, L.small_max};
  for (int i = 0; i < 4; ++i) if (b[i] > L.small_max) b[i] = L.small_max;
  for (int i = 0; i < 4; ++i) for (int j = i + 1; j < 4; ++j) if (b[j] < b[i]) { size_t t = b[i]; b[i] = b[j]; b[j] = t; }
  int rows = 0;
// ... 117 lines not shown
__attribute__((visibility("hidden"))) int bn254_pair_leaf_floor(size_t n, Ws ws, hipStream_t s, int mode);
__attribute__((visibility("hidden"))) int bn254_pair_fe_program(size_t n, Ws ws, const unsigned char* prog, hipStream_t s);
__attribute__((visibility("hidden"))) int bn254_pair_final_exp_product(size_t n, size_t k, Ws ws, uint8_t* gt_out, uint8_t* status_out, int raw_only,
                                                                       hipStream_t s);
__attribute__((visibility("hidden"))) int bn254_pair_final_exp(size_t n, Ws ws, int use_hash, uint8_t* status_out, const uint32_t* map,
                                                               const uint32_t* count, hipStream_t s, size_t base = 0);
__attribute__((visibility("hidden"))) int bn254_pair_miller_rand(size_t n, size_t n_groups, int items_per_pair, Ws ws, size_t gbase, hipStream_t s);
__attribute__((visibility("hidden"))) int bn254_pair_rand_tail(size_t n_groups, Ws ws, size_t gbase, hipStream_t s);
struct AggdSlots { const uint32_t* slot_agg; const uint64_t* incl; const uint64_t* lo; const uint64_t* hi; };
__attribute__((visibility("hidden"))) int bn254_pair_aggd_miller(size_t n_slots, Ws ws, AggdSlots sl, size_t gbase, size_t pbase, uint32_t* pseg, int last,
                                                                 hipStream_t s);
__attribute__((visibility("hidden"))) int bn254_pair_aggd_level(size_t n_elems, Ws ws, const uint32_t* seg, size_t ebase, size_t gbase, size_t pbase,
                                                                 uint32_t* pseg, int last, hipStream_t s);
__attribute__((visibility("hidden"))) int bn254_pair_aggd_tail(size_t n, Ws ws, size_t gbase, size_t obase, hipStream_t s);
__attribute__((visibility("hidden"))) int bn254_pair_aggregate(const uint32_t* tuple_msg, const uint64_t* tuple_off, const uint32_t* signer_idx, size_t n,
                                                               size_t n_signers, size_t n_msgs, Pool pk_pool, Pool sig_pool, Pool h_pool, Pool sub_pool,
                                                               size_t n_groups, Pool sub1_pool, size_t groups4, Ws ws, hipStream_t s,
                                                               const uint32_t* perm = nullptr, const Pool* wide2_pool = nullptr,
                                                               const Pool* wide1_pool = nullptr);
__attribute__((visibility("hidden"))) int bn254_pair_g2_mul_fixed(const uint8_t* d_scalars, size_t n, int reduce, Pool comb, uint8_t* d_out, uint8_t* d_status,
                                                                  hipStream_t s);
#define BN_G2_COMB_RECORDS (65 * 8 + 1)
__attribute__((visibility("hidden"))) int bn254_pair_g1_mul_fixed(const uint8_t* d_scalars, size_t n, int reduce, Pool comb, uint8_t* d_out, uint8_t* d_status,
                                                                  hipStream_t s);
#define BN_G1_COMB_RECORDS (65 * 8 + 3)
__attribute__((visibility("hidden"))) int bn254_pair_decode_g2(const uint8_t* pts, size_t n, uint32_t flags, Ws ws, int accumulate, hipStream_t s);
__attribute__((visibility("hidden"))) int bn254_pair_decompress_g2(const uint8_t* in, size_t n, Ws ws, hipStream_t s, int skip_subgroup_test = 0);

#define BN_KEY_LINE_WORDS (2 * 2 * BN_LIMBS)
struct KeyTable { const int32_t* lines; const uint8_t* st; const uint8_t* inf; uint32_t n_keys; };
__attribute__((visibility("hidden"))) int bn254_lm_miller_verify_keyed(size_t n, Ws ws, const uint32_t* key_idx, KeyTable kt, hipStream_t s);
__attribute__((visibility("hidden"))) int bn254_pair_miller_verify_keyed(size_t n, Ws ws, const uint32_t* key_idx, KeyTable kt, hipStream_t s, size_t base = 0,
                                                                         const uint32_t* map = nullptr, const uint32_t* count = nullptr);
#define AGGD_KEYED_W1_MAX_SLOTS 65536
__attribute__((visibility("hidden"))) int bn254_pair_aggd_keyed(size_t n_slots, int width, Ws ws, AggdSlots sl, const uint32_t* key_idx, KeyTable kt,
                                                                size_t gbase, size_t pbase, uint32_t* pseg, int last, hipStream_t s);
__attribute__((visibility("hidden"))) int bn254_pair_aggd_move(size_t n, Ws ws, size_t gbase, hipStream_t s);
#define AGG_RAND_MIN_PAIRS_DEFAULT 65536
#define AGG_RAND_GROUP_PAIRS_DEFAULT 1024
#define AGGR_SUM_WG 256
#define AGGR_PART_WORDS (3 * BN_LIMBS)
struct AggrScale { const uint32_t* pair_agg; const uint32_t* key_idx; const uint8_t* key_inf; const uint64_t* lo; uint32_t* nagg; uint32_t* ebkt;
                   uint64_t* cnt; uint64_t G; uint32_t n_keys; };
struct AggrSum { const uint32_t* perm; const uint64_t* tp; uint32_t* bkey; size_t m, gbase, cbase, tbase; uint32_t n_keys; };
__attribute__((visibility("hidden"))) int bn254_aggr_scale(size_t m, size_t n, Ws ws, size_t gbase, AggrScale a, const uint32_t* seed_be, int mode,
                                                           hipStream_t s);
__attribute__((visibility("hidden"))) int bn254_aggr_scatter(size_t n_entries, const uint32_t* ebkt, uint64_t* start, uint32_t* perm, uint32_t* eseg,
                                                             size_t n_b, uint32_t n_keys, const uint64_t* cnt, uint64_t* tp, hipStream_t s);
__attribute__((visibility("hidden"))) int bn254_aggr_glimits(size_t n_groups, uint32_t n_keys, size_t tbase, const uint64_t* cnt, const uint64_t* tp,
                                                             uint64_t* glo, uint64_t* ghi, Ws ws, size_t cbase, hipStream_t s);
__attribute__((visibility("hidden"))) int bn254_aggr_sum(size_t n_elems, int level0, Ws ws, AggrSum a, const uint32_t* seg_in, const int32_t* part_in,
                                                         uint32_t* pseg_out, int32_t* part_out, int last, hipStream_t s);
__attribute__((visibility("hidden"))) int bn254_aggr_collect(size_t n, Ws ws, size_t gbase, const uint64_t* lo, uint64_t G, const uint32_t* nagg,
                                                             const uint8_t* gst, uint8_t* status, uint8_t* queued, size_t n_groups, const uint64_t* glo,
                                                             const uint64_t* ghi, uint32_t* stats, hipStream_t s);
__attribute__((visibility("hidden"))) int bn254_pair_aggd_keyed_queued(size_t n_slots, int width, Ws ws, AggdSlots sl, const uint32_t* key_idx, KeyTable kt,
                                                                       size_t gbase, size_t pbase, uint32_t* pseg, int last, const uint8_t* queued,
                                                                       hipStream_t s);

#define BITMAP_TABLE_MAX_KEYS_DEFAULT 4096
struct BmKeysArg { const int32_t* xy; const uint8_t* st; const uint8_t* inf; const uint32_t* bad; uint32_t n_keys; };
__attribute__((visibility("hidden"))) int bn254_pair_bitmap_sum(const uint32_t* d_bits, size_t bm_words, size_t n, BmKeysArg keys, const int32_t* rec,
                                                                const uint8_t* rec_inf, Ws ws, hipStream_t s);

#define BITMAP_RAND_MIN_TUPLES_DEFAULT 81920
#define BITMAP_RAND_MAX_KEYS_DEFAULT 256
#define BITMAP_RAND_GROUP_TUPLES_DEFAULT 4096
#define COLLECT_WAVE_MIN_SHARES_DEFAULT 16
#define COLLECT_RAND_MIN_SHARES_DEFAULT 65664
#define COLLECT_RAND_MIN_PER_KEY_DEFAULT 42
#define COLLECT_OPT_MIN_SHARES_DEFAULT 1539
#define COLLECT_OPT_MIN_TUPLE_SHARES_DEFAULT 1
#define MERGE_WAVE_MIN_PARTS_DEFAULT 16
__attribute__((visibility("hidden"))) int bn254_aggd_scan_add(hipStream_t s, const uint64_t* in, size_t n, uint64_t* out, uint64_t* tot);
__attribute__((visibility("hidden"))) int bn254_aggd_scan_max(hipStream_t s, const uint64_t* in, size_t n, uint64_t* out, uint64_t* tot);
__attribute__((visibility("hidden"))) int bn254_aggd_keyed_slot_map(hipStream_t s, size_t n, const uint64_t* lo, const uint64_t* hi, int width,
                                                                    uint64_t* kincl, uint64_t* tot, size_t n_slots, uint32_t* slot_agg);

#define KEY_DEDUP_MAX_KEYS_DEFAULT 1024
#define KEY_DEDUP_MIN_MULT_DEFAULT 16
#define KEY_DEDUP_MAX_KEYS_LIMIT 16384
#define KD_MAX_PROBES 64u
#define KD_EMPTY 0xFFFFFFFFu
enum { KD_OVERFLOW = 1, KD_DEGENERATE = 2 };
enum { KD_CTL_D = 0, KD_CTL_FLAGS, KD_CTL_KEYED_N, KD_CTL_GENERIC_N, KD_CTL_BUILD, KD_CTL_HITS, KD_CTL_DROPPED, KD_CTL_WORDS = 8 };
enum { KD_DROP_CAPACITY = 1, KD_DROP_RESET = 2 };
struct KeyDedup {
  uint32_t* table;
  uint32_t* slot_id;
  uint32_t* slot_of;
  uint32_t* key_idx;
  uint32_t* rep;
  uint32_t* ctl;
  int32_t* lines;
  int32_t* c2;
  uint8_t* st;
  uint8_t* inf;
  uint32_t* row_of;
  uint32_t* build_row;
  uint32_t* build_rep;
  uint32_t* c_keys;
  uint32_t* c_index;
  uint32_t* c_state;
  uint32_t slot_mask, hash_mask, max_keys, min_mult, index_mask;
};
__attribute__((visibility("hidden"))) int bn254_kd_enqueue(const uint8_t* d_pks, size_t n, uint32_t flags, KeyDedup kd, int force_generic, int cache_reset,
                                                           int cache_on, hipStream_t s);
#define KD_BYTES_PER_ITEM ((size_t)(2 * 4 + 2) * sizeof(uint32_t))
#define KD_BYTES_PER_KEY ((size_t)BN_N_FIXED_LINES * (BN_KEY_LINE_WORDS + 2 * BN_LIMBS) * sizeof(int32_t) + (4 + 32 + 4) * sizeof(uint32_t) + 2)

__attribute__((visibility("hidden"))) int bn254_trio_miller_verify(size_t n, Ws ws, hipStream_t s, int mode = 0);
__attribute__((visibility("hidden"))) int bn254_quad_miller_verify(size_t n, Ws ws, hipStream_t s, int mode = 0);
__attribute__((visibility("hidden"))) int bn254_w8_miller_verify(size_t n, Ws ws, hipStream_t s, int mode = 0);
__attribute__((visibility("hidden"))) bool bn254_trio_fits_device();
__attribute__((visibility("hidden"))) bool bn254_quad_fits_device(int eight_waves);
__attribute__((visibility("hidden"))) int bn254_trio_final_exp(size_t n, Ws ws, int use_hash, uint8_t* status_out, hipStream_t s);
__attribute__((visibility("hidden"))) bool bn254_lm_fits_device();
__attribute__((visibility("hidden"))) int bn254_lm_miller_verify(size_t n, Ws ws, hipStream_t s, int mode = 0);
__attribute__((visibility("hidden"))) int bn254_lm_g2_subgroup(size_t n, Ws ws, hipStream_t s, int fail_status = 4 );
__attribute__((visibility("hidden"))) bool bn254_nonet_fits_device();
__attribute__((visibility("hidden"))) int bn254_nonet_final_exp(size_t n, Ws ws, int use_hash, uint8_t* status_out, hipStream_t s, int wide = 0);
__attribute__((visibility("hidden"))) int bn254_nonet_final_exp_product(size_t n, size_t k, Ws ws, uint8_t* gt_out, uint8_t* status_out, hipStream_t s);
#endif
```

### bn254_amd/csrc/gen_constants.py

```python
#!/usr/bin/env python3
import os

U = 4965661367192848881
Q = 36 * U**4 + 36 * U**3 + 24 * U**2 + 6 * U + 1
R_ORDER = 36 * U**4 + 36 * U**3 + 18 * U**2 + 6 * U + 1
LIMB_BITS = 29
N_LIMBS = 9
MONT_R = 1 << (LIMB_BITS * N_LIMBS)
XI = (9, 1)
G2X = (10857046999023057135944570762232829481370756359578518086990519993285655852781,
       11559732032986387107991004021392285783925812861821192530917403151452391805634)
G2Y = (8495653923123431417604973247489272438418190587263600148770280649306958101930,
       4082367875863433681332203403145435568316851327593401208105741076214120093531)


def add(a, b): return ((a[0] + b[0]) % Q, (a[1] + b[1]) % Q)
def sub(a, b): return ((a[0] - b[0]) % Q, (a[1] - b[1]) % Q)
def neg(a): return ((-a[0]) % Q, (-a[1]) % Q)
def mul(a, b): return ((a[0] * b[0] - a[1] * b[1]) % Q, (a[0] * b[1] + a[1] * b[0]) % Q)
def sqr(a): return mul(a, a)
def smul(a, k): return ((a[0] * k) % Q, (a[1] * k) % Q)
def conj(a): return (a[0], (-a[1]) % Q)


# ... 380 lines not shown
            return (c, (0,) + ds)
        cand = None
        for d in DSET:
            for sd in (d, -d):
                if m == sd:
                    r = (1, (sd,))
                elif abs((m - sd) // 2) < abs(m):
                    c, ds = best((m - sd) // 2)
                    r = (c + 1, (sd,) + ds)
                else:
                    continue
                if cand is None or r[0] < cand[0] or (r[0] == cand[0] and len(r[1]) < len(cand[1])):
                    cand = r
        return cand
    nz, digs = best(U)
    w4 = list(reversed(digs))
    while w4[0] == 0:
        w4.pop(0)
    assert sum(d << (len(w4) - 1 - i) for i, d in enumerate(w4)) == U and w4[0] > 0 and nz == 12
    o.append("#define BN_U_W4_LEN %d" % len(w4))
    o.append("BN_CONST signed char C_U_W4[BN_U_W4_LEN] = {%s};  /* signed digits of u from {0, +-1, +-15, +-19}, MSB first, %d non-zero */" %
             (", ".join(str(d) for d in w4), sum(1 for d in w4 if d)))
    for name, (code, slots) in (("CHECK", fe_program_check(w4)), ("EXACT", fe_program_exact(w4))):
        o.append("#define BN_FE_%s_LEN %d" % (name, len(code)))
        o.append("#define BN_FE_%s_SLOTS %d" % (name, len(slots)))
        o.append("BN_CONST unsigned char C_FE_%s[BN_FE_%s_LEN][2] = {%s};  /* accumulator-machine program of the final exponentiation (gen_constants.py: fe_program_%s; %s) */" %
                 (name, name, ", ".join("{%d, %d}" % ins for ins in code), name.lower(),
                  ", ".join("%d %s" % (sum(1 for op, _ in code if op == k), FE_OPNAMES[k]) for k in range(1, 8))))
    o.append("/* line coefficients (c0 -> *yP, c1 -> *xP, c2 == 1) for Q = -G2::one(), in order of use */")
    o.append("BN_CONST int32_t C_NEG_G2_LINES[BN_N_FIXED_LINES][3][2][BN_LIMBS] = {")
    for ln in lines:
        o.append("  {%s, %s, %s}," % (c_fp2(ln[0]), c_fp2(ln[1]), c_fp2(ln[2])))
    o.append("};")
    o.append("")
    path = os.path.join(here, "bn254_constants.h")
    with open(path, "w") as f:
        f.write("\n".join(o))
    print("wrote", path, "lines:", len(lines), "naf weight:", sum(1 for d in naf if d))


if __name__ == "__main__":
    main()
```

### bn254_amd/engine.py

```python
import ctypes

from . import _native

G1_BYTES, G2_BYTES, GT_BYTES, SCALAR_BYTES = 64, 128, 384, 32
FLAG_G2_SUBGROUP_CHECK = 1
FLAG_REJECT_IDENTITY = 2
FLAG_RAND64 = 0x100
FLAG_RAND_GLV = 0x200
OPT_SPLIT_MILLER = 1
OPT_HASH_MAX_TRIES = 2
OPT_RAND_ITEMS_PER_LANE = 3
OPT_PAIR_LANES = 4
OPT_RAND_MIN_BATCH = 5
OPT_TRIO_MAX_BATCH = 6
OPT_HASH_DIRECT_WIDTH = 7
OPT_TRIO_WAVE_ROLES = 8
OPT_AGG_SUBSET_MIN_TUPLES = 9
OPT_CLOCK_PROBE = 10
OPT_AGG_SORT_BY_MSG = 11
OPT_PINNED_STAGING = 12
OPT_NONET_MAX_BATCH = 13
OPT_LM_MAX_BATCH = 15
OPT_NONET_WIDE = 16
OPT_AGG_WIDE_MIN_TUPLES = 14
OPT_MAX_CHUNK = 17
OPT_ASSUME_FREE_MB = 18
OPT_G2_FIXED_BASE = 19
OPT_KEY_DEDUP = 20
OPT_KEY_DEDUP_MAX_KEYS = 21
OPT_KEY_DEDUP_MIN_MULT = 22
OPT_KEY_DEDUP_FORCE_GENERIC = 23
OPT_KEY_DEDUP_HASH_BITS = 24
OPT_AGGD_KEYED_ROUTE = 25
OPT_AGG_RAND_MIN_PAIRS = 26
OPT_AGG_RAND_GROUP_PAIRS = 27
OPT_BITMAP_TABLE_MAX_KEYS = 28
OPT_BITMAP_ROUTE = 29
OPT_HASH_SCHEDULE = 30
OPT_HASH_WIDE_WIDTH = 31
OPT_HASH_TAIL_CHUNK = 32
OPT_BITMAP_RAND_MIN_TUPLES = 33
OPT_BITMAP_RAND_GROUP_TUPLES = 34
OPT_BITMAP_RAND_MAX_KEYS = 35
OPT_KEY_CACHE = 36
OPT_COLLECT_RAND_MIN_SHARES = 38
OPT_COLLECT_RAND_MIN_PER_KEY = 39
COLLECT_RAND_MIN_SHARES_DEFAULT = 65664
COLLECT_RAND_MIN_PER_KEY_DEFAULT = 42
OPT_COLLECT_OPT_MIN_SHARES = 40
OPT_AGG_T4_ROUTE = 42
OPT_COLLECT_OPT_MIN_TUPLE_SHARES = 41
COLLECT_OPT_MIN_SHARES_DEFAULT = 1539
COLLECT_OPT_MIN_TUPLE_SHARES_DEFAULT = 1
OPT_MERGE_WAVE_MIN_PARTS = 43
MERGE_WAVE_MIN_PARTS_DEFAULT = 16
OPT_COLLECT_WAVE_MIN_SHARES = 37


class NativeError(RuntimeError):

    def __init__(self, fn, rc):
        what = "HIP error %d" % (-rc) if -10000 < rc < 0 else {-10001: "bad argument", -10002: "misaligned device pointer",
                                                                -10003: "no HIP device (bn254_amd has no CPU fallback)"}.get(rc, "error")
        super().__init__("%s failed: %s (rc=%d)" % (fn, what, rc))
        self.rc = rc


def _check(fn, rc):
    if rc != 0:
        raise NativeError(fn, rc)


def pack_messages(messages):
    n = len(messages)
    off = (ctypes.c_uint64 * (n + 1))()
    pos = 0
# ... 42 lines not shown
        _check("bn254_ctx_expect_msgs_len", self._lib.bn254_ctx_expect_msgs_len(self._h, int(msgs_len)))

    def set_option(self, option, value):
        _check("bn254_ctx_set_option", self._lib.bn254_ctx_set_option(self._h, option, value))

    def probe_issue_rate(self, op, waves_per_simd=2):
        rate, simds = ctypes.c_double(0), ctypes.c_int(0)
        _check("bn254_probe_issue_rate", self._lib.bn254_probe_issue_rate(self._h, op, waves_per_simd, ctypes.byref(rate), ctypes.byref(simds)))
        return rate.value, simds.value

    def route_table(self):
        m, a, b = (ctypes.c_uint64 * 8)(), (ctypes.c_int * 8)(), (ctypes.c_int * 8)()
        rows = self._lib.bn254_debug_route_table(self._h, m, a, b, 8)
        if rows < 0:
            _check("bn254_debug_route_table", rows)
        return [(int(m[i]), int(a[i]), int(b[i])) for i in range(rows)]

    def debug_key_dedup_last(self):
        o = (ctypes.c_uint32 * 5)()
        _check("bn254_debug_key_dedup_last", self._lib.bn254_debug_key_dedup_last(self._h, o))
        return dict(zip(("ran", "keys", "flags", "keyed_n", "generic_n"), (int(x) for x in o)))

    def debug_key_cache_last(self):
        o = (ctypes.c_uint32 * 5)()
        _check("bn254_debug_key_cache_last", self._lib.bn254_debug_key_cache_last(self._h, o))
        return dict(zip(("ran", "keys", "hits", "built", "dropped"), (int(x) for x in o)))

    def debug_key_tables(self, which, first, count):
        words = (ctypes.c_int32 * (count * 87 * 36))()
        rep = (ctypes.c_uint32 * max(count, 1))()
        st, inf = ctypes.create_string_buffer(max(count, 1)), ctypes.create_string_buffer(max(count, 1))
        _check("bn254_debug_key_tables", self._lib.bn254_debug_key_tables(self._h, which, first, count, words, rep, st, inf))
        return list(words), (list(rep)[:count] if which == 0 else None), st.raw[:count], inf.raw[:count]

    def debug_agg_tables_info(self):
        o = (ctypes.c_uint64 * 5)()
        _check("bn254_debug_agg_tables", self._lib.bn254_debug_agg_tables(self._h, -1, 0, 0, o, None))
        return dict(zip(("n_groups", "groups4", "wide2", "wide1", "t4_builder"), (int(v) for v in o)))

    def debug_agg_tables(self, which, first, count):
        size = 128 if which in (0, 3, 5) else 64
        pts, fl = ctypes.create_string_buffer(max(count * size, 1)), ctypes.create_string_buffer(max(count, 1))
        _check("bn254_debug_agg_tables", self._lib.bn254_debug_agg_tables(self._h, which, first, count, pts, fl))
        return pts.raw[:count * size], fl.raw[:count]

    def debug_agg_rand_last(self):
        o = (ctypes.c_uint64 * 6)()
        _check("bn254_debug_agg_rand_last", self._lib.bn254_debug_agg_rand_last(self._h, o))
        return dict(zip(("ran", "groups", "table_pairs", "failed_groups", "rechecked", "single_groups"), (int(x) for x in o)))

    def debug_agg_rand_sums(self):
        return self._debug_rand_sums("bn254_debug_agg_rand_sums")

    def _debug_rand_sums(self, name):
        f = getattr(self._lib, name)
        dims = (ctypes.c_uint64 * 2)()
        _check(name, f(self._h, dims, 0, 0, None, None, None, None, None, None))
        ng, ntp = int(dims[0]), int(dims[1])
        if ng == 0:
            return []
        nagg, verdict, s = (ctypes.c_uint32 * ng)(), ctypes.create_string_buffer(ng), ctypes.create_string_buffer(64 * ng)
        first, keys, pts = (ctypes.c_uint64 * (ng + 1))(), (ctypes.c_uint32 * max(ntp, 1))(), ctypes.create_string_buffer(64 * max(ntp, 1))
        _check(name, f(self._h, dims, ng, ntp, nagg, verdict, s, first, keys, pts))
        assert (int(dims[0]), int(dims[1])) == (ng, ntp)
        return [dict(nagg=int(nagg[g]), verdict=verdict.raw[g], s=s.raw[64 * g:64 * g + 64],
                     pairs=[(int(keys[t]), pts.raw[64 * t:64 * t + 64]) for t in range(int(first[g]), int(first[g + 1]))]) for g in range(ng)]
# ... 654 lines not shown
```

### include/bn254_hip.h

```cpp
#ifndef BN254_HIP_H
#define BN254_HIP_H

#include <stddef.h>
#include <stdint.h>

#ifdef __cplusplus
extern "C" {
#endif

typedef struct bn254_ctx bn254_ctx;

#define BN254_FLAG_G2_SUBGROUP_CHECK 1u
#define BN254_FLAG_REJECT_IDENTITY 2u
#define BN254_FLAG_RAND64 0x100u
#define BN254_FLAG_RAND_GLV 0x200u

#define BN254_E_BAD_ARGUMENT (-10001)
#define BN254_E_MISALIGNED (-10002)
#define BN254_E_NO_DEVICE (-10003)
#define BN254_E_RCCL (-10004)
#define BN254_E_NO_MEMORY (-10005)

#define BN254_OK 0
#define BN254_ERR_HASH_TO_POINT 1
// ... 226 lines not shown
                                   const uint8_t *const *d_sigs, const uint8_t *const *d_pks, size_t n , uint32_t flags,
                                   uint8_t *const *d_status_all , void *const *streams );
int bn254_mgpu_batch_verify_compressed(bn254_mgpu *mg, const uint8_t *msgs, const uint64_t *msg_off, const uint8_t *sigs33, const uint8_t *pks65,
                                       size_t n, uint8_t *status);
int bn254_mgpu_register_keys(bn254_mgpu *mg, const uint8_t *pks , size_t n_keys, uint32_t flags, uint8_t *key_status );
int bn254_mgpu_batch_verify_keyed(bn254_mgpu *mg, const uint8_t *msgs, const uint64_t *msg_off, const uint8_t *sigs, const uint32_t *key_idx, size_t n,
                                  uint32_t flags, uint8_t *status);
int bn254_mgpu_batch_aggregate_verify(bn254_mgpu *mg, const uint8_t *msgs, const uint64_t *msg_off, size_t n_msgs, const uint8_t *pk_pool,
                                      size_t n_signers, const uint8_t *sig_pool, const uint32_t *tuple_msg, const uint64_t *tuple_off,
                                      const uint32_t *signer_idx, size_t n, uint32_t flags, uint8_t *status);
int bn254_mgpu_batch_pairing(bn254_mgpu *mg, const uint8_t *g1 , const uint8_t *g2 , size_t n, size_t k,
                             uint32_t flags, uint8_t *gt , uint8_t *status , uint64_t *checksum );
int bn254_mgpu_batch_pairing_device(bn254_mgpu *mg, const uint8_t *const *d_g1, const uint8_t *const *d_g2, size_t n, size_t k,
                                    uint32_t flags, uint8_t *const *d_gt, uint8_t *const *d_status_all, uint64_t *const *d_checksum,
                                    void *const *streams);
int bn254_mgpu_batch_hash_to_g1(bn254_mgpu *mg, const uint8_t *msgs, const uint64_t *msg_off, size_t n, uint8_t *points ,
                                uint8_t *status , uint8_t *tries );

#ifndef BN254_NO_DEV_HOOKS
#define BN254_OPT_SPLIT_MILLER 1
#define BN254_OPT_PAIR_LANES 4
#define BN254_OPT_RAND_ITEMS_PER_LANE 3
#define BN254_OPT_TRIO_WAVE_ROLES 8
#define BN254_OPT_HASH_DIRECT_WIDTH 7
#define BN254_OPT_HASH_SCHEDULE 30
#define BN254_OPT_HASH_WIDE_WIDTH 31
#define BN254_OPT_HASH_TAIL_CHUNK 32
#define BN254_OPT_NONET_WIDE 16
#define BN254_OPT_AGG_SORT_BY_MSG 11
#define BN254_OPT_CLOCK_PROBE 10
#define BN254_OPT_HASH_MAX_TRIES 2
#define BN254_OPT_G2_FIXED_BASE 19
#define BN254_OPT_KEY_DEDUP_FORCE_GENERIC 23
#define BN254_OPT_KEY_DEDUP_HASH_BITS 24
#define BN254_OPT_AGGD_KEYED_ROUTE 25
#define BN254_OPT_AGG_RAND_GROUP_PAIRS 27
#define BN254_OPT_BITMAP_RAND_GROUP_TUPLES 34
#define BN254_OPT_BITMAP_ROUTE 29
#define BN254_OPT_AGG_T4_ROUTE 42
#define BN254_OPT_ASSUME_FREE_MB 18
int bn254_debug_route_table(bn254_ctx *ctx, uint64_t *max_n, int *miller, int *fe, int cap);
int bn254_debug_key_dedup_last(bn254_ctx *ctx, uint32_t out[5]);
int bn254_debug_key_cache_last(bn254_ctx *ctx, uint32_t out[5]);
int bn254_debug_key_tables(bn254_ctx *ctx, int which, size_t first, size_t count, int32_t *lines, uint32_t *rep, uint8_t *st, uint8_t *inf);
int bn254_debug_agg_tables(bn254_ctx *ctx, int which, size_t first, size_t count, uint8_t *points, uint8_t *flags);
int bn254_debug_agg_rand_last(bn254_ctx *ctx, uint64_t out[6]);
int bn254_debug_agg_rand_sums(bn254_ctx *ctx, uint64_t dims[2], size_t group_cap, size_t pair_cap, uint32_t *nagg, uint8_t *verdict,
                              uint8_t *s_g , uint64_t *first_pair , uint32_t *pair_key, uint8_t *pair_point );
int bn254_debug_collect_rand_last(bn254_ctx *ctx, uint64_t out[4]);
int bn254_debug_collect_opt_last(bn254_ctx *ctx, uint64_t out[4]);
int bn254_debug_bitmap_rand_last(bn254_ctx *ctx, uint64_t out[6]);
int bn254_debug_bitmap_rand_sums(bn254_ctx *ctx, uint64_t dims[2], size_t group_cap, size_t pair_cap, uint32_t *nagg, uint8_t *verdict,
                                 uint8_t *s_g , uint64_t *first_pair , uint32_t *pair_key, uint8_t *pair_point );
int bn254_debug_fp_op(bn254_ctx *ctx, int op, const uint8_t *a, const uint8_t *b, size_t n, uint8_t *out, uint8_t *status);
int bn254_debug_fp12_op(bn254_ctx *ctx, int op, const uint8_t *a, const uint8_t *b, size_t n, uint8_t *out);
int bn254_debug_final_exp_limbs(bn254_ctx *ctx, int layout, const int32_t *limbs , size_t n, uint8_t *gt ,
                                uint8_t *status );
int bn254_debug_hash_candidate(bn254_ctx *ctx, const uint8_t *h , size_t n, uint8_t *out , uint8_t *status);
int bn254_debug_miller_loop(bn254_ctx *ctx, const uint8_t *g1, const uint8_t *g2, size_t n, uint8_t *f );

int bn254_probe_issue_rate(bn254_ctx *ctx, int op, int waves_per_simd, double *wave_inst_per_s, int *n_simd);
int bn254_probe_leaf_floor(bn254_ctx *ctx, size_t n, int mode, float *ms);
int bn254_probe_fe_program(bn254_ctx *ctx, size_t n, const uint8_t *prog, size_t n_steps, float *ms);
#endif

#ifdef __cplusplus
}
#endif
#endif
```

Baseline: 15.87 million.

## Precompute folded line-pair products per deduplicated key for Miller loop

For keyed batch verify, each NAF nonzero step's two fixed-Q lines are pre-multiplied into five Fp2 coefficient rows (K0..K4) per key and for the constant -G2 generator, stored in a new fold table. The keyed Miller loop then multiplies by a single folded line product instead of two separate sparse line multiplications at those steps. This cuts Fp12 multiplication work in the Miller loop. The cost is extra per-key precompute and memory for the folded tables, plus more constant-memory traffic. It is enabled by default through a new option.

```diff
diff --git a/bn254_amd/_native.py b/bn254_amd/_native.py
--- a/bn254_amd/_native.py
+++ b/bn254_amd/_native.py
@@ -98,6 +98,8 @@
         L.bn254_debug_key_cache_last.argtypes = [vp, ctypes.POINTER(ctypes.c_uint32)]
     if hasattr(L, "bn254_debug_key_tables"):
         L.bn254_debug_key_tables.argtypes = [vp, i32, sz, sz, vp, vp, vp, vp]
+    if hasattr(L, "bn254_debug_key_fold_tables"):
+        L.bn254_debug_key_fold_tables.argtypes = [vp, sz, sz, vp]
     if hasattr(L, "bn254_debug_agg_tables"):
         L.bn254_debug_agg_tables.argtypes = [vp, i32, sz, sz, vp, vp]
     L.bn254_debug_agg_rand_last.argtypes = [vp, ctypes.POINTER(ctypes.c_uint64)]
@@ -209,7 +211,7 @@
     "bn254_batch_g1_add", "bn254_batch_g2_add", "bn254_batch_g1_mul", "bn254_batch_g2_mul", "bn254_batch_g1_mul_device",
     "bn254_batch_g2_mul_device", "bn254_batch_sign", "bn254_batch_sign_device", "bn254_batch_g1_sum", "bn254_batch_g2_sum",
     "bn254_batch_aggregate_verify", "bn254_batch_aggregate_verify_device", "bn254_ctx_register_pools", "bn254_ctx_register_pools_device",
-    "bn254_batch_aggregate_verify_registered", "bn254_batch_aggregate_verify_registered_device", "bn254_batch_aggregate_verify_distinct", "bn254_batch_aggregate_verify_distinct_device", "bn254_batch_aggregate_verify_distinct_keyed", "bn254_batch_aggregate_verify_distinct_keyed_device", "bn254_batch_aggregate_verify_distinct_keyed_randomized", "bn254_batch_aggregate_verify_distinct_keyed_randomized_device", "bn254_batch_g1_decompress", "bn254_batch_g2_decompress", "bn254_debug_fp_op", "bn254_debug_fp12_op", "bn254_debug_final_exp_limbs", "bn254_debug_miller_loop", "bn254_debug_hash_candidate", "bn254_debug_route_table", "bn254_debug_key_dedup_last", "bn254_debug_key_cache_last", "bn254_debug_key_tables", "bn254_debug_agg_tables", "bn254_debug_agg_rand_last", "bn254_debug_agg_rand_sums", "bn254_probe_issue_rate", "bn254_probe_leaf_floor", "bn254_probe_fe_program", "bn254_ctx_set_profiling", "bn254_ctx_last_kernel_ms", "bn254_ctx_set_option", "bn254_ctx_last_clocks", "bn254_ctx_expect_msgs_len", "bn254_ctx_register_keys", "bn254_batch_verify_keyed", "bn254_batch_verify_keyed_device", "bn254_batch_verify_keyed_randomized", "bn254_batch_verify_keyed_randomized_device",
+    "bn254_batch_aggregate_verify_registered", "bn254_batch_aggregate_verify_registered_device", "bn254_batch_aggregate_verify_distinct", "bn254_batch_aggregate_verify_distinct_device", "bn254_batch_aggregate_verify_distinct_keyed", "bn254_batch_aggregate_verify_distinct_keyed_device", "bn254_batch_aggregate_verify_distinct_keyed_randomized", "bn254_batch_aggregate_verify_distinct_keyed_randomized_device", "bn254_batch_g1_decompress", "bn254_batch_g2_decompress", "bn254_debug_fp_op", "bn254_debug_fp12_op", "bn254_debug_final_exp_limbs", "bn254_debug_miller_loop", "bn254_debug_hash_candidate", "bn254_debug_route_table", "bn254_debug_key_dedup_last", "bn254_debug_key_cache_last", "bn254_debug_key_tables", "bn254_debug_key_fold_tables", "bn254_debug_agg_tables", "bn254_debug_agg_rand_last", "bn254_debug_agg_rand_sums", "bn254_probe_issue_rate", "bn254_probe_leaf_floor", "bn254_probe_fe_program", "bn254_ctx_set_profiling", "bn254_ctx_last_kernel_ms", "bn254_ctx_set_option", "bn254_ctx_last_clocks", "bn254_ctx_expect_msgs_len", "bn254_ctx_register_keys", "bn254_batch_verify_keyed", "bn254_batch_verify_keyed_device", "bn254_batch_verify_keyed_randomized", "bn254_batch_verify_keyed_randomized_device",
     "bn254_batch_verify_keyed_bitmap", "bn254_batch_verify_keyed_bitmap_device",
     "bn254_batch_verify_keyed_bitmap_randomized", "bn254_batch_verify_keyed_bitmap_randomized_device", "bn254_debug_bitmap_rand_last",
     "bn254_debug_bitmap_rand_sums", "bn254_batch_collect_keyed_bitmap", "bn254_batch_collect_keyed_bitmap_device",
diff --git a/bn254_amd/csrc/bn254_constants.h b/bn254_amd/csrc/bn254_constants.h
--- a/bn254_amd/csrc/bn254_constants.h
+++ b/bn254_amd/csrc/bn254_constants.h
@@ -169,3 +169,29 @@
   {{{-162397500, 2954997, 152488182, -65669248, -2226221, 126434462, 136504248, -45920178, 1018187}, {37038594, -230220348, -39757353, 51278743, 94503435, 69559177, 117383119, -38335104, 1747986}}, {{-168849216, 266245294, 103631925, -116049438, -183139901, -68554844, 259384813, -968803, 1609363}, {215323032, -48099119, -244987994, -57467655, -73007447, -145862608, -75994125, -187878897, 359235}}, {{-176370655, -199481511, -128831276, 21759002, 178483129, -45989682, -237679608, 86689705, 903222}, {0, 0, 0, 0, 0, 0, 0, 0, 0}}},
   {{{198924502, -95920802, 109010388, 97989720, -212428967, 216061620, -144460110, 93801757, 1223757}, {-249735650, 57427941, 134749786, -254932027, 35573088, 90419683, 133149999, 143547148, 125881}}, {{194882581, 87312206, -43835174, -161184211, 204737166, -171525322, -265395304, 139734743, 2318771}, {-210600565, -38893026, 17554950, -242192057, 58146045, -142126381, 157173323, 44273995, 2017346}}, {{-176370655, -199481511, -128831276, 21759002, 178483129, -45989682, -237679608, 86689705, 903222}, {0, 0, 0, 0, 0, 0, 0, 0, 0}}},
 };
+#define BN_N_FOLD_ROWS 22
+BN_CONST unsigned char C_FOLD_FIRST[BN_N_FOLD_ROWS] = {0, 3, 8, 11, 16, 19, 22, 26, 33, 37, 40, 44, 50, 53, 58, 61, 65, 70, 74, 77, 80, 85};
+BN_CONST int32_t C_NEG_G2_FOLD[BN_N_FOLD_ROWS][5][2][BN_LIMBS] = {
+  {{{-53926915, 23356922, 194139575, -115411448, 214488792, -107049629, -8576688, -87923000, 131312}, {251271253, 228551138, -50838115, 226760741, 70526116, -177103959, 118020308, -13900495, 1342359}}, {{198518913, 18340493, 227742623, -173891007, -119174917, 70612499, 174155627, 35462283, 2622874}, {258760290, -229893025, -261123530, -198909900, 12593688, 156918972, 80695314, -247576648, 1461938}}, {{-57592009, 266293567, 165435136, -96924786, -133734097, 164830367, 111470088, -252907886, 714228}, {51366545, -19388777, 240753571, -101044389, -239886304, 127492939, 248343859, -226887004, 993365}}, {{-29415806, -75776099, -143811338, 84452418, -238648986, 61416779, -263109307, 78320750, 1888334}, {24612542, 190918295, 23060281, 147578244, 242436372, -186088598, 180177203, 42900993, 594800}}, {{-130186793, 69604189, 171708848, -130126856, -180299376, -38321142, 250170482, 32545852, 388892}, {-61945987, 197310945, 241577428, 122768735, -91077879, 2599338, -233920866, 249856380, 507340}}},
+  {{{209073893, 55166304, -61921313, 159036095, -258520773, 185338765, 152983764, -261376030, 64047}, {-180361504, 184382653, -261032720, -101372833, -7235641, -226826515, 140110803, 88321284, 2221309}}, {{-16377450, 104807868, -34040336, -260663281, -216104816, 3932846, 41667067, -198480287, 1102006}, {241450924, -265270766, -158712996, -222356769, -31110450, -256012515, 141091258, -178357368, 2236664}}, {{-95667758, 7535389, 256085616, 61649804, 13064093, 124716735, 73801931, 19823655, 1872194}, {-185914751, -134594435, 1207445, 213891560, -45373413, 250335233, 71476717, -163989967, 1082976}}, {{-14860166, 167792817, 50057247, -142978543, -185517827, -4583319, -229634492, -170597581, 1584435}, {264488959, 140567133, 77132379, -264429639, -75855472, 27872417, -251809036, 199664729, 191358}}, {{-9769281, -203999705, -198707561, 114711948, -119537815, -231308863, 144909415, -179361623, 2904869}, {-146088511, 128599479, 73275017, 215566896, 239608457, -138109749, 90813385, -268098787, 828688}}},
+  {{{-130419860, 211551546, -212755485, 203808607, 150779948, -268186322, -117038852, -241213478, 1587821}, {96603635, 196843936, 213897727, 211290287, -58235825, -60221038, 98196329, 45570077, 2410921}}, {{-35350769, -184485500, -93729520, 244014179, 208570557, 170485372, -111871807, 160808285, 1318540}, {267809414, 219352661, 77049756, -137253859, 40938643, -167512594, -211419085, -164000331, 435171}}, {{-20409384, -258365279, 229937997, -186542934, -88729244, -102088979, 79435933, -208222788, 1949875}, {39307050, 20231863, 72298810, -96891754, -50730343, 243637973, 89239901, -84823181, 1165404}}, {{-77141371, -238187031, -68668932, -99506418, -21932446, 241227644, 106536394, 239816616, 1566397}, {188720895, -188440158, 30991308, -195611539, 74529450, -137911862, 211237789, -121281862, 207279}}, {{83878893, -216544482, 169605161, 32932816, -228164128, -112681886, -193957794, 79173486, 277126}, {14892851, 113457495, -213762532, -149090213, -141965832, -66628852, 242965762, 185802489, 44340}}},
+  {{{259429827, -75610747, -104521406, 212051599, -133677191, 260306193, 228078547, -244364819, 2144337}, {-203678357, 183453524, 30568942, -127241309, 88061595, 30530918, -146543179, 254965230, 1724506}}, {{88694078, -232111328, -99313224, 64813159, -67466415, -80214634, -198934016, -263229017, 1654783}, {258603500, -166305941, 167730862, -231002900, -76927367, 91980181, -208625326, 15075499, 1208208}}, {{-100017792, -32358950, 183129140, -184017788, -51828768, -174221137, -126656894, 76183147, 1609164}, {-228266101, 89543718, -44884523, -69754899, -131140901, -198018923, -136383885, -137044920, 1199659}}, {{86557565, 138313264, -217653971, -200047563, -108495944, 117482788, 208962576, 221290064, 1425865}, {-155508464, 267874079, -208066408, -200646564, -130966225, 140362578, 53407253, 22041687, 2699379}}, {{115385457, -171547781, -225977000, -241806006, 47379038, -32321524, 188229882, 215227692, 418991}, {-16746174, -265925849, 147789462, -142796745, -177758116, -220533541, 243063819, -126860123, 2624633}}},
+  {{{104435028, 200335436, 227915151, -223881731, -5732294, -145887533, -188340374, -183745069, 1551440}, {119363630, -29288881, 70041675, -128935245, -251961512, 132506475, 206390444, -72090122, 319721}}, {{259539054, -262230812, 5059525, -258820359, -62444945, -197128693, -150576410, -253093523, 1247468}, {-23764138, 33895737, 80884000, 268051025, -153372290, 208661143, 193308080, -170789595, 1740819}}, {{-64783066, -12357825, 77219060, -235229088, 16461002, -118377628, 88396651, 256604253, 1329991}, {-262540763, -103164113, 69188726, -234119869, -156620612, -235886504, -141788371, -234460820, 2372035}}, {{-106618330, -145951334, 128928750, 105619292, -188774015, 57526800, -141452541, -200793501, 1553062}, {-93062457, 65952181, -200231068, -28782033, -193815207, 260137542, 204434802, -230205308, 401039}}, {{-84440317, 43306834, -174718354, 268361358, -129789038, 226302456, 55774935, -95277835, 2745014}, {-78380854, 106292011, -53015387, -118118105, 35771716, 215187520, -106314482, -100291649, 3163594}}},
+  {{{-259682409, 205059046, -130538633, -138942372, 41782671, 147002051, -215986410, -171332501, 2595742}, {-428728, -112346322, -201534476, 170188116, -158006451, 248040308, 201260606, 24474185, 111346}}, {{-93998212, -107064933, 261117322, 31052560, 140236469, -175226027, 88760545, 45812356, 2393578}, {167471666, 183333630, 73208695, 63014059, 265098229, -242914515, 221475783, -62712723, 1052924}}, {{184384134, 223513479, -220589075, 30348806, -63339092, -207211686, -235746221, 220613593, 1899908}, {105795006, -248996898, -55110555, 193596822, 7536177, -26212942, 151176220, -227005399, 1187601}}, {{161036069, 176651699, -37094420, 129690540, 29007941, 144563013, -134597929, 175457308, 348981}, {100329215, -55022289, -14235885, 204528890, -220141493, 171103737, 151839219, -107682856, 1347276}}, {{-33188553, -43376329, -117480253, 641272, -35925145, -227921294, -39887336, -118230103, 395888}, {-216012908, -17609015, 133395710, -244574073, -107628197, -97407631, -215469350, 229104213, 1761114}}},
+  {{{-95206519, -59847406, 64447069, 32274315, -248772148, -192081003, 198242023, 74227806, 3168293}, {-264239559, 177009366, 138315733, -109219552, 199106547, 33025948, 75686531, -254881359, 112755}}, {{79095162, 94560571, 168286406, 73803021, 214117392, -162955972, -257522927, 174607818, 839599}, {-92297806, 132289069, 240051056, -59233350, 138755467, -234840328, 184780338, -6795630, 443933}}, {{198057203, -151073860, 126020756, 118693627, -120326012, -204146859, 190498416, -151978663, 608961}, {-134030870, 104918830, 177940693, 247409108, 78260013, 244128513, 140584603, -24270349, 617097}}, {{246873076, 109559276, 67351309, 267012208, -120345456, -216939372, -114961167, 165830549, 524602}, {-172167144, -259268803, -149149046, -104352635, -239954908, 200811263, 201081411, -43655268, 1583492}}, {{-160205725, 176313273, 190194359, -205793320, 28002710, 59766154, 183979445, -225436162, 2621094}, {-96329176, 23516022, -153931956, 38218053, -210400765, 155244265, -158084620, 262878779, 2823580}}},
+  {{{-58200121, -128069830, -144449525, -56843566, -83262078, -10324324, 204504961, -214093782, 2511108}, {-56850967, -147202179, -40218420, -104733474, -234314364, -174807498, 54703209, -139774287, 1573378}}, {{-213533077, 242303454, 260934220, 74098349, 249137411, -166462885, -252082851, -11569932, 2988268}, {-46559327, 68790647, -8106896, 83607256, 239574258, -832175, -226303161, -237757277, 228138}}, {{-102799002, -141001282, -65323924, 224554794, 607807, -249387361, -254526318, -66577440, 1199613}, {-29430704, -148267146, 135908018, 56903136, 57400501, 8199880, -224564297, -205725468, 509393}}, {{156388049, 129009395, 90471824, -14882068, -194860512, -221902687, -220871213, 84056706, 1349016}, {92308943, -151425345, 225936043, 20321518, -352478, 14259886, 256041900, 261758018, 163424}}, {{-122460315, -145878404, -167476038, 115567051, 207731691, 164189538, 236312515, 196697436, 676615}, {-224252407, 65516874, -155248037, 127697401, -180557611, -142725889, -9663404, 176978439, 2781616}}},
+  {{{82904438, 181065266, 248793007, -221902848, 171286300, 31400991, -250826313, -127386437, 2933552}, {-238905417, -7147178, 184914312, 97510174, -148686954, 64981196, 77780542, 83665296, 529581}}, {{235079927, 61434756, 141310728, -16882454, 226968749, -84215099, 19700217, 213322745, 1870988}, {131276899, -184652224, 84206827, 153022560, 10127424, 44867719, 144956158, 223031110, 1614725}}, {{231008778, -257761710, 29948328, 192893730, 238403028, -59287468, 254499321, -165067151, 2657001}, {-77623901, -138796826, 105337675, -1550433, 217499741, -202632236, -114468073, -2514384, 97387}}, {{-94279328, -264444780, -110738230, -215703188, 93025975, -24645901, -68652199, 211101205, 3111495}, {137503319, 19994616, -247043303, -191641815, -202830859, 75586288, -102009824, 110962879, 816736}}, {{73995704, -75059446, 248523230, 244483234, 24125732, 238977385, 111775937, 169493632, 169751}, {189708382, -11153151, -39786974, 78760442, 50233788, -267772229, -123632828, 248377814, 411296}}},
+  {{{-157940632, -13817589, -164214402, 123554333, 248093248, -131950031, -87546103, -47962386, 557357}, {129013445, -149556371, 89954612, -163733335, 174731216, 39815215, 24187, 235725693, 2289842}}, {{-164962473, -212595483, -244784660, -90802440, 257885457, 116292158, 164992313, -151410440, 1540888}, {-217489167, 255629210, -126981658, -180707711, -10595093, -62794484, 43402101, -241491443, 770811}}, {{-73952229, -165753357, -19867705, 49899591, -82627818, 75808297, 115415281, 248945473, 2384152}, {-20587099, 147224624, 186708393, -10180264, 111970302, 118115792, -230535868, 190862775, 781777}}, {{-142548463, 259336945, 178142765, 209089194, 171253586, 216203357, 16657340, 207205629, 636331}, {223246169, 261619191, -249501271, 107559847, 159947095, 173859451, -240323491, 195836685, 2512961}}, {{-218291578, -234018528, 449125, -134217559, 121421777, 132723891, 113606503, 99335649, 2251264}, {264234355, 256483186, 104932049, -189543398, -230680255, -223453744, 219869489, -148798397, 2868502}}},
+  {{{-27104189, -89580870, 260876561, 93067155, 266959916, -98104019, 37572267, -184218160, 665429}, {-163870855, -38532344, -101134974, -245964597, 207376932, 250077540, 44960688, -121453535, 1657882}}, {{49506228, 168634929, 102996897, 213156381, 221424753, 30661481, 164397149, 242074176, 2404811}, {-9446608, -40992251, -59352361, -52268696, -224979409, -267984966, -105913193, 260943433, 463529}}, {{-115242631, -20049242, 142719668, -49658081, 78604101, -245067823, 61449933, 57388510, 1936480}, {-131455747, -170952600, 138014574, -231619147, -67838959, 67523915, -67825565, -164325518, 1311293}}, {{-266569576, -221200573, 256552644, 195619419, 163256274, -123362043, 178554721, 159790407, 326083}, {-53317418, -144655767, 48919056, -8365512, 120021982, 106222355, -142036866, 64693849, 2636220}}, {{-10188918, -46448206, -227726210, 65892000, 163252805, 115212425, 214022431, 170476574, 360395}, {-142691758, -27999514, 120842790, 73874818, 206352546, -79703395, 209835556, -211021975, 879683}}},
+  {{{231322686, -190583818, -250512141, 91482864, -68382290, 138766313, -227823068, -38471339, 3096806}, {-58681559, -205948256, -237136552, 255782817, 107623807, -245882793, -102109783, 205732773, 1802245}}, {{177872086, 265374798, 37377066, 27354116, 263464637, 178777288, 153540517, 134300563, 3171094}, {-261849934, -81156328, 173714377, -131431173, -152126185, 156586501, 132507537, 225962256, 840913}}, {{9992018, -98054113, 242759626, -22744940, -250568431, -197636261, -238702470, 163645062, 2546539}, {182567513, 110930241, 128627065, 28585582, 13096934, -245039225, -96266450, 141170476, 3169533}}, {{169149580, 123459544, 35505259, -202301124, -152752783, 252995600, 151798883, -224255126, 893931}, {203455852, 58037725, -121437406, 235359607, 132194682, -183843433, -117382718, 116906, 959710}}, {{-82229094, -234165576, -154573990, -113531496, -22343773, 29925402, 246554678, 215253098, 274675}, {-3420469, 58842074, -198299582, -113737521, 221117765, -195131865, 58592932, 217917480, 1388284}}},
+  {{{-117888837, -194495599, -241128777, 136751064, -209848238, -12170827, 250610960, 70142862, 346504}, {202025934, 132450756, -118742481, -193680979, -55601992, 153116454, -72928406, -236694476, 542688}}, {{27355730, -110452777, -131645734, -138050825, -106466672, -265321819, 42736407, 177439958, 1785356}, {74118618, -101518966, -38364607, -262837866, -182936659, 249384036, 138932328, -57476758, 2271567}}, {{155029449, -83387895, -25701161, 236652146, 128047386, -233298956, 170387121, 156141972, 629882}, {-158279117, -78514154, -137041575, 216157634, 47566800, 23054640, -110329723, -241909252, 1285497}}, {{-105368788, -185395992, 234961852, -128112212, 14509809, 147758541, -34584575, -258444408, 1863083}, {-63097673, 100240932, 197411773, 168852787, 144402864, -243367000, 57738288, -18488719, 15950}}, {{223973817, -231191948, 2779710, -241019550, 7311510, 258046020, -59829494, -153875855, 1171488}, {178749350, -28815000, -13378333, -216405378, -246639713, -266276415, 263951114, 28472400, 2534956}}},
+  {{{84289506, -86265549, 40498582, 184409234, 166441687, 21659170, -98151840, -177608792, 2214871}, {186864406, -196428218, -62191690, 105877495, -251499277, 245584230, -142188914, -228320798, 1272195}}, {{-252084769, -115778279, -56362708, -247314159, -54305580, 89578961, -133340920, 81620997, 631343}, {259826557, -36849018, 116326167, 236728929, 131509258, -34243840, -12963592, -33682493, 1422077}}, {{-177069722, 25293284, 266270268, -174510351, 171291220, -114602977, -260363255, 214406693, 2852988}, {105298063, -9705446, 199939197, 40555178, -103942543, -47401051, -92392401, -43744474, 2806126}}, {{60926780, 234983350, 131343379, -107110301, 253090756, -61626272, 215412521, -68914309, 1325686}, {43283240, 258792101, 259125002, -74434349, -79440750, 237202321, -32004488, 104569217, 1530770}}, {{-62821736, -105921108, 166635938, -264138035, -41044422, -32567282, -1687722, 254041303, 2553100}, {219589069, 249134603, -7080183, 231870736, 149839184, 51967110, -152011260, 183548229, 616170}}},
+  {{{165859153, 144244287, -98494731, 47366673, -33956883, 240867799, -209742691, 72894566, 366686}, {-26876893, -52289214, 141848069, -83120029, 36219687, -235059657, -105393162, 244516158, 1674392}}, {{-258831541, -109970025, 234433347, 18819986, 107765667, 131432938, 240754085, -115036469, 896793}, {-71756496, -152130551, 173335040, 168671049, -199719830, 257606634, -256441854, 47328062, 2171750}}, {{-223535504, 75708855, 80679738, -60101679, 176900676, 268392977, 143380337, 210374397, 1374364}, {-263799662, -26836606, 152414631, -255620489, 113037952, 68947126, 17109673, -114440735, 1989931}}, {{-86175899, -41205427, 5171770, 247374949, -66086820, -219035133, -21869390, -27318996, 1719456}, {-94949049, -149879027, -139343431, 58409214, 111265978, 109909243, 101207690, 28373930, 361854}}, {{60025631, 222020991, -130964161, -228648257, 252312852, -18249027, -262734744, 214988660, 3023809}, {92435914, 253885570, 59807586, -182877823, 73331403, -191310251, 235346763, -102507307, 884447}}},
+  {{{-49655495, -62210747, -104732288, -239115456, 87208597, -169352444, 232608887, -188941280, 1978622}, {-80171926, -109085679, -220190138, -132262722, 247806478, 185929360, -174981813, 96191030, 514829}}, {{47569711, -265983393, -123073755, -5361976, -120639393, -37194195, -105322267, 128653773, 2373568}, {171433797, -236045043, 165576160, 43947138, -105727831, 182475246, 89821784, 143054052, 419526}}, {{-100990345, -96243893, -165239660, -164337479, 17336380, -85703977, -129193131, 24587452, 2220469}, {-41630197, 175964866, -59109118, 256184133, 1285922, -94428375, -256475177, -221943583, 844704}}, {{71692883, 42266145, -226340696, 139610222, 89872251, 181440787, -229416834, -86003623, 3143860}, {20266273, -235402571, 214776741, 168424439, -17019229, -252161802, -54585304, 239447374, 1021715}}, {{-52348943, 154340129, 115957005, -14791531, -148001012, -154240848, 151074370, 250791001, 2108942}, {-56323991, 78641166, -90517077, -180569614, 4549508, 103161422, 142730193, 129974258, 467303}}},
+  {{{-249209121, 73554231, 5918850, 162011761, -21363011, -232689217, 180152724, -48122584, 1755710}, {48649104, -90966414, 208458459, 178714535, -6098825, 122938278, -103526002, -186796139, 2773198}}, {{191005089, -29579860, -218338066, -50873020, -199048630, 5069870, 71694202, -246846529, 2428246}, {-178888262, 140790869, -98402146, 15973811, 199912660, 248940658, -258304573, 191771610, 2200302}}, {{-235304633, -108271898, 139576888, -113418729, 131089628, -214831740, -44213964, -236020574, 2236613}, {-176901852, 111211416, -91550492, 102433163, -222404441, -20915754, -93295500, 158397531, 516794}}, {{-93830414, -241059631, -258573974, -114467708, 190262948, -63048659, 43935217, 52901107, 1355922}, {152661240, -211239850, -82118462, 108419721, 60509106, 159588014, 123497865, 151969383, 2412727}}, {{150758903, -88209847, -208628687, 212212486, -139536582, 155986039, -12404312, 68124370, 2354959}, {74396246, -44299433, 217880550, 264706614, 94128675, -146542796, -167064699, -105270644, 1543028}}},
+  {{{-176935358, 147196411, 156341278, -18626400, -129160322, 204511891, -261191672, -197786504, 105396}, {-34098299, 213548305, -146766424, 169340306, 250355902, -127894031, -160440116, 186445579, 1462470}}, {{-33038717, 148516216, 227689948, -254312325, -228756529, 167452132, 34676703, -183810364, 1065478}, {-247637162, 69129241, -31928992, -221123618, 4761525, -166529552, -206903231, 62081218, 2523519}}, {{-124742584, -159032791, -22671252, -260257634, 177675659, 228202038, 250921194, -23871591, 2484066}, {-13769555, -231193117, 217340113, -193798204, -257104672, -259206028, -99121109, -175081158, 752290}}, {{-130400195, -48377577, -171547588, 60646231, 222100437, -208566020, -110151693, 181654578, 2875053}, {-143579428, -174917901, -80141686, -71140571, -149101371, -76763374, 84319350, 231732744, 1788242}}, {{-172485526, -94993573, -255551147, -192891046, 247316486, -27841830, -225347412, -54890544, 995130}, {-188877157, -125679193, -41540793, 2564996, -228551778, -243271717, -97528509, -175137252, 387547}}},
+  {{{-256830952, -51848306, 82703985, -118377458, 161917454, -95479134, 142759207, 256509572, 486181}, {-248748707, -59951285, -195258778, 117667144, 63621988, -133675394, 14907992, 264923280, 3058716}}, {{27305719, -162455958, 17546630, 49170271, -258945781, 176765814, -204634203, -2208213, 1064998}, {128776547, -227484848, -100295555, -153158208, 122290903, 43933631, -160907606, 53686967, 1481769}}, {{245255341, 195661093, 11441220, 24978317, 203050742, -216219421, -122016149, 199486206, 2351475}, {-261233022, -141349887, -128546913, -63513501, 122514628, -226268420, -104671485, 220524275, 587979}}, {{177528158, -238450535, -227318194, -130752158, -160941977, 90985374, 224973414, -190145601, 627088}, {-116291268, 122592311, 243212609, -235589067, 147730404, 82504561, -22979824, -265125973, 571334}}, {{106634158, 113525303, 115863397, 198256247, -40932839, 168970149, 130589211, -159124234, 2238152}, {133823250, 264701168, -117432760, 19084725, -129180600, -91819034, 116313177, 135421784, 2326952}}},
+  {{{41664399, 244912742, -253897310, 177416979, 53462330, 221960011, 22104048, -94593022, 901028}, {-226494579, 221263713, -249876682, -18257734, 14487606, -124906900, 206435851, -42151367, 311802}}, {{50067815, 23627301, -35107125, -241808992, -91884368, 128285459, -37899656, -168085752, 2853816}, {-184536500, -193643829, -263057747, -143724797, -31979220, -231656308, 150207909, -179865312, 1285923}}, {{-161818209, -56074201, 230366246, -111319105, -108787613, -258438414, -92893668, -17076851, 1184595}, {-77883598, 31761449, -192245723, 163414427, 222359812, -174526470, -165940815, 247057907, 1890130}}, {{-164886841, 80287265, -88347936, -243060418, -184061023, -193269095, 182405143, -116856286, 2655850}, {-225717626, 214291463, -230204243, -81433088, 22920951, 129613539, -238015990, -151871649, 308180}}, {{106334188, 228665793, 154933627, -91515147, -221994159, 92405668, 172449585, 96791155, 195987}, {-179676521, -136665392, 21200409, -96673596, -128891980, -97155509, -250524939, 26872799, 2797332}}},
+  {{{-266425167, -265250780, -236848977, 219422083, -158323325, 36796480, 162857887, 49742566, 838615}, {-248283559, -86985053, -108100364, -38870978, 40932246, 228484570, 117416348, -56144274, 3164032}}, {{266566127, 34766671, 97715653, 83455487, 99680880, -205883723, 245748899, -156104926, 3089611}, {-193807421, 187869013, 197243171, -105707141, 236346457, -122432443, 183310379, 59932426, 1227027}}, {{-76025801, 26132452, -186617045, 97248896, -146733271, 21801266, -99111534, -136901690, 2230337}, {-34837243, 232476885, -229923095, -242038994, 187038242, -181772215, 194782979, -147063990, 1354118}}, {{84824344, -238776740, -163041776, 28270281, 177176451, -143354163, 232903666, 13266439, 1775487}, {151665666, 69563942, -156446750, 235350908, 115262410, -79332168, -91763868, 263852290, 3064794}}, {{-95570627, 254320322, -195379101, 204958981, -8813268, 227994057, 138489411, -200008046, 2014641}, {-131262681, 52073199, 261870066, 131938030, 55411291, 51206417, -221694080, 134034283, 2788376}}},
+  {{{111060989, -244666275, 197440947, 130175447, -184271117, -187565012, -223431457, -182214321, 2012250}, {-229255541, 261009399, -161934562, -185995261, -243931546, -259975990, 238769704, -216320166, 1489689}}, {{-267887804, 126740294, 55251544, 61577294, -127712441, -125498543, 169485050, -73624711, 1173195}, {-216955078, -45364624, -169753260, -235723868, 17566705, -142310326, 209442473, 37632961, 1771126}}, {{182086781, 102156988, -55471737, -72376654, -226172016, -99965130, 118784829, 65338054, 1578710}, {7212371, -186984753, -142626752, -75509134, -202103166, 191750445, -51466081, -40640739, 1082464}}, {{36527002, -92965805, 261498570, 32320472, -214655188, -194374830, -7955861, 47881579, 2241944}, {-212697056, -172792407, 94992433, -203653284, 130076523, 159978860, 250533118, 105212044, 1873867}}, {{152059790, -200377531, 119392705, 212114750, 197374680, 248867353, -16947133, -102154176, 756728}, {4722467, -86992145, -227433044, 237211200, -14861403, 248881923, 81179197, -143604902, 2376581}}},
+};
diff --git a/bn254_amd/csrc/bn254_devhooks.hip b/bn254_amd/csrc/bn254_devhooks.hip
--- a/bn254_amd/csrc/bn254_devhooks.hip
+++ b/bn254_amd/csrc/bn254_devhooks.hip
@@ -248,6 +248,29 @@
   if (inf) HIP_TRY(hipMemcpy(inf, src_inf + first, count, hipMemcpyDeviceToHost));
   return 0;
 }
+int bn254_debug_key_fold_tables(bn254_ctx* c, size_t first, size_t count, int32_t* rows_out) {
+  if (!c || !rows_out) return BN254_E_BAD_ARGUMENT;
+  HIP_TRY(hipSetDevice(c->device));
+  HIP_TRY(hipDeviceSynchronize());
+  const size_t per_key = (size_t)BN_N_FOLD_ROWS * BN_KEY_FOLD_WORDS;
+  uint32_t ctl[KD_CTL_WORDS];
+  if (!c->kd_last_run || !c->kd_ctl || !c->kd_fold_last) return BN254_E_BAD_ARGUMENT;
+  HIP_TRY(hipMemcpy(ctl, c->kd_ctl, sizeof ctl, hipMemcpyDeviceToHost));
+  if (first + count > ctl[KD_CTL_D] || first + count > c->kd_keys_cap) return BN254_E_BAD_ARGUMENT;
+  if (ctl[KD_CTL_BUILD] + ctl[KD_CTL_HITS] != ctl[KD_CTL_D]) return BN254_E_BAD_ARGUMENT;
+  if (count == 0) return 0;
+  uint32_t* rows = (uint32_t*)malloc(count * sizeof(uint32_t));
+  if (!rows) return BN254_E_NO_MEMORY;
+  hipError_t e = hipMemcpy(rows, c->kd_row_of_last + first, count * sizeof(uint32_t), hipMemcpyDeviceToHost);
+  int rc = e == hipSuccess ? 0 : -(int)e;
+  for (size_t k = 0; k < count && !rc; ++k) {
+    if (rows[k] >= c->kd_keys_cap) { rc = BN254_E_BAD_ARGUMENT; break; }
+    e = hipMemcpy(rows_out + k * per_key, c->kd_fold_last + (size_t)rows[k] * per_key, per_key * sizeof(int32_t), hipMemcpyDeviceToHost);
+    if (e != hipSuccess) rc = -(int)e;
+  }
+  free(rows);
+  return rc;
+}
 static int debug_rand_last(bn254_ctx* c, int ran, const uint32_t* stats, uint64_t out[6]) {
   if (!c || !out) return BN254_E_BAD_ARGUMENT;
   for (int i = 0; i < 6; ++i) out[i] = 0;
diff --git a/bn254_amd/csrc/bn254_hip.hip b/bn254_amd/csrc/bn254_hip.hip
--- a/bn254_amd/csrc/bn254_hip.hip
+++ b/bn254_amd/csrc/bn254_hip.hip
@@ -448,6 +448,7 @@
     c->kd_items_cap = c->kd_keys_cap = 0;
     c->kd_ctl = nullptr;
     c->kd_lines_last = nullptr;
+    c->kd_fold_last = nullptr;
     c->kd_cache_valid = false;
     if (hipMalloc((void**)&c->kd_buf, items_cap * KD_BYTES_PER_ITEM + keys_cap * KD_BYTES_PER_KEY + 512) != hipSuccess) {
       (void)hipGetLastError();
@@ -466,7 +467,8 @@
   kd.slot_of = (uint32_t*)take(c->kd_items_cap * 4);
   kd.key_idx = (uint32_t*)take(c->kd_items_cap * 4);
   kd.lines = (int32_t*)take(c->kd_keys_cap * BN_N_FIXED_LINES * BN_KEY_LINE_WORDS * 4);
-  kd.c2 = (int32_t*)take(c->kd_keys_cap * BN_N_FIXED_LINES * 2 * BN_LIMBS * 4);
+  kd.fold = (int32_t*)take(c->kd_keys_cap * KD_FOLD_KEY_WORDS * 4);
+  kd.c2 = kd.fold;
   kd.rep = (uint32_t*)take(c->kd_keys_cap * 4);
   kd.ctl = (uint32_t*)take(KD_CTL_WORDS * 4);
   c->kd_ctl = kd.ctl;
@@ -481,7 +483,7 @@
   kd.c_index = (uint32_t*)take(4 * c->kd_keys_cap * 4);
   kd.c_state = (uint32_t*)take(4);
   kd.index_mask = (uint32_t)(index_slots - 1);
-  c->kd_lines_last = kd.lines; c->kd_rep_last = kd.rep; c->kd_st_last = kd.st; c->kd_inf_last = kd.inf; c->kd_row_of_last = kd.row_of;
+  c->kd_lines_last = kd.lines; c->kd_fold_last = kd.fold; c->kd_rep_last = kd.rep; c->kd_st_last = kd.st; c->kd_inf_last = kd.inf; c->kd_row_of_last = kd.row_of;
   kd.slot_mask = (uint32_t)(slots - 1);
   kd.hash_mask = c->kd_hash_bits > 0 && c->kd_hash_bits < 32 ? (1u << c->kd_hash_bits) - 1 : 0xFFFFFFFFu;
   kd.max_keys = (uint32_t)keys;
@@ -718,6 +720,7 @@
   c->key_dedup = 1;
   c->kd_max_keys = KEY_DEDUP_MAX_KEYS_DEFAULT;
   c->kd_min_mult = KEY_DEDUP_MIN_MULT_DEFAULT;
+  c->kd_fold = KEY_DEDUP_FOLD_DEFAULT;
   c->kd_cache = 1;
   c->bm_table_max_keys = BITMAP_TABLE_MAX_KEYS_DEFAULT;
   c->device = hip_device;
@@ -878,6 +881,7 @@
   if (option == BN254_OPT_KEY_DEDUP) { if (value < 0 || value > 1) return BN254_E_BAD_ARGUMENT; c->key_dedup = value; return 0; }
   if (option == BN254_OPT_KEY_DEDUP_MAX_KEYS) { if (value < 0 || value > KEY_DEDUP_MAX_KEYS_LIMIT) return BN254_E_BAD_ARGUMENT; c->kd_max_keys = value; return 0; }
   if (option == BN254_OPT_KEY_DEDUP_MIN_MULT) { if (value < 1) return BN254_E_BAD_ARGUMENT; c->kd_min_mult = value; return 0; }
+  if (option == BN254_OPT_KEY_DEDUP_FOLD) { if (value < 0 || value > 1) return BN254_E_BAD_ARGUMENT; c->kd_fold = value; return 0; }
   if (option == BN254_OPT_KEY_DEDUP_FORCE_GENERIC) { c->kd_force_generic = value == 2 ? 2 : value != 0; return 0; }
   if (option == BN254_OPT_KEY_CACHE) { if (value < 0 || value > 1) return BN254_E_BAD_ARGUMENT; c->kd_cache = value; c->kd_cache_valid = false; return 0; }
   if (option == BN254_OPT_KEY_DEDUP_HASH_BITS) { if (value < 0 || value > 32) return BN254_E_BAD_ARGUMENT; c->kd_hash_bits = value; return 0; }
@@ -974,7 +978,9 @@
   if (kd) {
     HIP_TRY(hipStreamWaitEvent(s, c->kd_join, 0));
     const KeyTable kt = {kd->lines, kd->st, kd->inf, kd->max_keys};
-    if ((rc = bn254_pair_miller_verify_keyed(n, c->ws, kd->key_idx, kt, s, 0, nullptr, kd->ctl + KD_CTL_KEYED_N))) return rc;
+    if (c->kd_fold) rc = bn254_pair_miller_verify_keyed_fold(n, c->ws, kd->key_idx, kt, kd->fold, s, 0, nullptr, kd->ctl + KD_CTL_KEYED_N);
+    else rc = bn254_pair_miller_verify_keyed(n, c->ws, kd->key_idx, kt, s, 0, nullptr, kd->ctl + KD_CTL_KEYED_N);
+    if (rc) return rc;
     if ((rc = bn254_pair_miller_verify(n, c->ws, nullptr, kd->ctl + KD_CTL_GENERIC_N, s))) return rc;
     PROF_MARK(3);
     if ((rc = bn254_pair_final_exp(n, c->ws, 1, d_status, nullptr, nullptr, s))) return rc;
diff --git a/bn254_amd/csrc/bn254_host.h b/bn254_amd/csrc/bn254_host.h
--- a/bn254_amd/csrc/bn254_host.h
+++ b/bn254_amd/csrc/bn254_host.h
@@ -77,6 +77,7 @@
   int kd_max_keys;
   int kd_min_mult;
   int kd_force_generic;
+  int kd_fold;
   int kd_hash_bits;
   hipStream_t kd_stream;
   hipEvent_t kd_fork, kd_join;
@@ -89,6 +90,7 @@
   size_t kd_items_cap, kd_keys_cap;
   uint32_t* kd_ctl;
   const int32_t* kd_lines_last;
+  const int32_t* kd_fold_last;
   const uint32_t* kd_rep_last;
   const uint32_t* kd_row_of_last;
   const uint8_t *kd_st_last, *kd_inf_last;
diff --git a/bn254_amd/csrc/bn254_keydedup.h b/bn254_amd/csrc/bn254_keydedup.h
--- a/bn254_amd/csrc/bn254_keydedup.h
+++ b/bn254_amd/csrc/bn254_keydedup.h
@@ -52,6 +52,21 @@
 }
 #endif
 
+BN_DEV void kd_fold_pair(const Fp2& c0, const Fp2& c1, const Fp2& d0, const Fp2& d1, Fp2 k[5]) {
+  const Fp2 k0 = fp2_mul(c0, d0), k2 = fp2_mul(c1, d1);
+  const Fp2 k1 = fp2_sub(fp2_sub(fp2_mul(NS(294, fp2_add(c0, c1)), NS(295, fp2_add(d0, d1))), k0), k2);
+  const Fp2 k3 = fp2_add(c0, d0), k4 = fp2_add(c1, d1);
+  BN_FOR_ROLES(r) { k[0].c[r] = fp_canon(k0.c[r]); k[1].c[r] = fp_canon(k1.c[r]); k[2].c[r] = fp_canon(k2.c[r]); k[3].c[r] = fp_canon(k3.c[r]); k[4].c[r] = fp_canon(k4.c[r]); }
+}
+#if !defined(__HIPCC__)
+static inline void kd_fold_lines(const Fp2* c0, const Fp2* c1, Fp2 (*fold)[5]) {
+  for (int r = 0; r < BN_N_FOLD_ROWS; ++r) {
+    const int i = C_FOLD_FIRST[r];
+    kd_fold_pair(c0[i], c1[i], c0[i + 1], c1[i + 1], fold[r]);
+  }
+}
+#endif
+
 #if defined(__HIPCC__)
 BN_DEV bool load_fp_be_checked(Fp& r, const uint8_t* p, uint32_t& any) {
   const uint32_t* w = (const uint32_t*)p;
diff --git a/bn254_amd/csrc/bn254_keydedup.hip b/bn254_amd/csrc/bn254_keydedup.hip
--- a/bn254_amd/csrc/bn254_keydedup.hip
+++ b/bn254_amd/csrc/bn254_keydedup.hip
@@ -241,7 +241,7 @@
     for (int k = 0; k < 5; ++k) m.e[lv].w[k] = t[m.pair].w[k];
   }
   m.rows = kd.lines + (size_t)row * BN_N_FIXED_LINES * BN_KEY_LINE_WORDS;
-  m.c2s = kd.c2 + (size_t)row * BN_N_FIXED_LINES * 2 * BN_LIMBS;
+  m.c2s = kd.c2 + (size_t)row * KD_FOLD_KEY_WORDS;
   m.degenerate = false;
   KD_LM_FENCE();
   kd_builder_program(m);
@@ -259,7 +259,7 @@
   int32_t* row = kd.lines + ((size_t)j * BN_N_FIXED_LINES + (line ? p : 0u)) * BN_KEY_LINE_WORDS;
   {
     Fp2 leaf = fp2_one();
-    if (line) leaf = fp2_reduce_weak(kd_load_own(kd.c2 + ((size_t)j * BN_N_FIXED_LINES + p) * KD_NODE_WORDS));
+    if (line) leaf = fp2_reduce_weak(kd_load_own(kd.c2 + (size_t)j * KD_FOLD_KEY_WORDS + p * KD_NODE_WORDS));
     kd_store_own(prod + (KD_TREE_LEAVES + p) * KD_NODE_WORDS, leaf);
   }
   __syncthreads();
@@ -282,13 +282,25 @@
     }
     __syncthreads();
   }
-  if (!line) return;
-  const Fp2 c2inv = kd_load_own(inv + (KD_TREE_LEAVES + p) * KD_NODE_WORDS);
-  const Fp2 a = fp2_mul(kd_load_own(row), c2inv), b = fp2_mul(kd_load_own(row + 2 * BN_LIMBS), c2inv);
-  Fp2 r0, r1;
-  BN_FOR_ROLES(k) { r0.c[k] = fp_canon(a.c[k]); r1.c[k] = fp_canon(b.c[k]); }
-  kd_store_own(row, r0);
-  kd_store_own(row + 2 * BN_LIMBS, r1);
+  if (line) {
+    const Fp2 c2inv = kd_load_own(inv + (KD_TREE_LEAVES + p) * KD_NODE_WORDS);
+    const Fp2 a = fp2_mul(kd_load_own(row), c2inv), b = fp2_mul(kd_load_own(row + 2 * BN_LIMBS), c2inv);
+    Fp2 r0, r1;
+    BN_FOR_ROLES(k) { r0.c[k] = fp_canon(a.c[k]); r1.c[k] = fp_canon(b.c[k]); }
+    kd_store_own(row, r0);
+    kd_store_own(row + 2 * BN_LIMBS, r1);
+    kd_store_own(prod + (KD_TREE_LEAVES + p) * KD_NODE_WORDS, r0);
+    kd_store_own(inv + (KD_TREE_LEAVES + p) * KD_NODE_WORDS, r1);
+  }
+  __syncthreads();
+  if (p >= BN_N_FOLD_ROWS) return;
+  const uint32_t first = C_FOLD_FIRST[p];
+  Fp2 k[5];
+  kd_fold_pair(kd_load_own(prod + (KD_TREE_LEAVES + first) * KD_NODE_WORDS), kd_load_own(inv + (KD_TREE_LEAVES + first) * KD_NODE_WORDS),
+               kd_load_own(prod + (KD_TREE_LEAVES + first + 1) * KD_NODE_WORDS), kd_load_own(inv + (KD_TREE_LEAVES + first + 1) * KD_NODE_WORDS), k);
+  int32_t* frow = kd.fold + (size_t)j * KD_FOLD_KEY_WORDS + p * BN_KEY_FOLD_WORDS;
+#pragma unroll
+  for (int e = 0; e < 5; ++e) kd_store_own(frow + e * 2 * BN_LIMBS, k[e]);
 }
 KERNEL_KD void k_kd_decide(size_t n, KeyDedup kd, int force_generic, int cache_on) {
   const bool keyed = force_generic != 1 && kd_viable(kd, n) && (kd.ctl[KD_CTL_FLAGS] & KD_DEGENERATE) == 0;
diff --git a/bn254_amd/csrc/bn254_pair.hip b/bn254_amd/csrc/bn254_pair.hip
--- a/bn254_amd/csrc/bn254_pair.hip
+++ b/bn254_amd/csrc/bn254_pair.hip
@@ -180,6 +180,58 @@
 int bn254_pair_miller_verify_keyed(size_t n, Ws ws, const uint32_t* key_idx, KeyTable kt, hipStream_t s, size_t base, const uint32_t* map,
                                    const uint32_t* count) {
   k_miller_verify_keyed_pair<<<(unsigned)((2 * n + BN_PAIR_WG - 1) / BN_PAIR_WG), BN_PAIR_WG, 0, s>>>(n, ws, key_idx, kt, base, map, count);
+  HIP_TRY(hipGetLastError());
+  return 0;
+}
+struct WsMonomials {
+  int32_t* f0;
+  size_t stride;
+  uint32_t i;
+  __device__ __forceinline__ void uniform() {
+    f0 = (int32_t*)bn_wave_uniform(f0);
+    stride = ((size_t)(uint32_t)__builtin_amdgcn_readfirstlane((int)(uint32_t)(stride >> 32)) << 32) | (uint32_t)__builtin_amdgcn_readfirstlane((int)(uint32_t)stride);
+  }
+  __device__ __forceinline__ void put(int pair, int j, const Fp& x) {
+#pragma unroll
+    for (int k = 0; k < BN_LIMBS; ++k) f0[((size_t)(3 * pair + j) * BN_LIMBS + k) * stride + i] = x.v[k];
+  }
+  __device__ __forceinline__ Fp get(int pair, int j) const {
+    Fp r;
+#pragma unroll
+    for (int k = 0; k < BN_LIMBS; ++k) r.v[k] = f0[((size_t)(3 * pair + j) * BN_LIMBS + k) * stride + i];
+    return r;
+  }
+};
+KERNEL_PAIR void k_miller_verify_keyed_fold_pair(size_t n, Ws ws, const uint32_t* key_idx, KeyTable kt, const int32_t* fold, size_t base, const uint32_t* map,
+                                                 const uint32_t* count) {
+  size_t i = ((size_t)blockIdx.x * BN_PAIR_WG + threadIdx.x) >> 1;
+  if (i >= n) return;
+  if (count && i >= *count) return;
+  if (map) i = map[i];
+  uint32_t key = key_idx[i];
+  i += base;
+  uint8_t kst = ST_OK;
+  if (key >= kt.n_keys) { kst = ST_INDEX_OOB; key = 0; }
+  else kst = kt.st[key];
+  const bool key_inf = kst != ST_OK || kt.inf[key] != 0;
+  if ((threadIdx.x & 1u) == 0) {
+    const uint8_t prev = ws_byte(ws, BY_ST_DECODE, i);
+    ws_byte(ws, BY_ST_DECODE, i) = prev != ST_OK ? prev : kst;
+  }
+  G1Affine sig, h;
+  ws_load_g1(ws, PL_P1X, BY_P1_INF, i, sig);
+  ws_load_g1(ws, PL_P2X, BY_P2_INF, i, h);
+  __shared__ Fp12PairSlot lds_f[BN_PAIR_WG];
+  Fp12& f = lds_f[threadIdx.x].v;
+  const WsMonomials mono = {ws.planes + (size_t)PL_F0 * BN_LIMBS * ws.stride, ws.stride, (uint32_t)i};
+  BN_CLK_BEGIN(ws);
+  miller_loop_keyed_fold<true>(f, h, key_inf, kt.lines, fold, key, sig, mono);
+  BN_CLK_END(ws, 0);
+  ws_store_f12_own(ws, i, f);
+}
+int bn254_pair_miller_verify_keyed_fold(size_t n, Ws ws, const uint32_t* key_idx, KeyTable kt, const int32_t* fold, hipStream_t s, size_t base,
+                                        const uint32_t* map, const uint32_t* count) {
+  k_miller_verify_keyed_fold_pair<<<(unsigned)((2 * n + BN_PAIR_WG - 1) / BN_PAIR_WG), BN_PAIR_WG, 0, s>>>(n, ws, key_idx, kt, fold, base, map, count);
   HIP_TRY(hipGetLastError());
   return 0;
 }
diff --git a/bn254_amd/csrc/bn254_pairing.h b/bn254_amd/csrc/bn254_pairing.h
--- a/bn254_amd/csrc/bn254_pairing.h
+++ b/bn254_amd/csrc/bn254_pairing.h
@@ -202,6 +202,87 @@
   step();
   step();
 }
+#if defined(BN_SPLIT_FP2)
+#if defined(__HIPCC__)
+#define BN_MEMBER __device__ __forceinline__
+#else
+#define BN_MEMBER inline
+#endif
+struct G1MonomialValues {
+  Fp v[2][3];
+  BN_MEMBER void put(int pair, int j, const Fp& x) { v[pair][j] = x; }
+  BN_MEMBER Fp get(int pair, int j) const { return v[pair][j]; }
+  BN_MEMBER void uniform() {}
+};
+template <class Mono>
+BN_DEV void g1_monomials_put(Mono& mono, int pair, const G1Affine& p) {
+  BN_FOR_ROLES(k) {
+    mono.put(pair, 0, fp_sqr(p.x)); mono.put(pair, 1, fp_mul(p.x, p.y)); mono.put(pair, 2, fp_sqr(p.y));
+  }
+}
+struct LineProduct { Fp6 b0; Fp2 b10, b11; };
+template <int S, class Mono>
+BN_DEV void folded_row_product(LineProduct& L, const int32_t (*row)[2][BN_LIMBS], const G1Affine& p, const Mono& mono, int pair, bool skip, bool any_skip) {
+  L.b0.c0 = NS(S, fp2_add(fp2_mul_fp(fp2_load_const(row[0]), mono.get(pair, 2)), fp2_load_const(C_XI_MONT)));
+  L.b0.c1 = fp2_mul_fp(fp2_load_const(row[2]), mono.get(pair, 0));
+  L.b0.c2 = fp2_mul_fp(fp2_load_const(row[4]), p.x);
+  L.b10 = fp2_mul_fp(fp2_load_const(row[1]), mono.get(pair, 1));
+  L.b11 = fp2_mul_fp(fp2_load_const(row[3]), p.y);
+  if (any_skip) {
+    const Fp2 zero = fp2_zero();
+    L.b0.c0 = fp2_select(skip, fp2_one(), L.b0.c0);
+    L.b0.c1 = fp2_select(skip, zero, L.b0.c1);
+    L.b0.c2 = fp2_select(skip, zero, L.b0.c2);
+    L.b10 = fp2_select(skip, zero, L.b10);
+    L.b11 = fp2_select(skip, zero, L.b11);
+  }
+}
+template <class T> BN_DEV const T* bn_wave_uniform(const T* p) {
+#if defined(__HIP_DEVICE_COMPILE__)
+  const uint64_t v = (uint64_t)p;
+  return (const T*)(((uint64_t)(uint32_t)__builtin_amdgcn_readfirstlane((int)(uint32_t)(v >> 32)) << 32) | (uint32_t)__builtin_amdgcn_readfirstlane((int)(uint32_t)v));
+#else
+  return p;
+#endif
+}
+template <bool F_LDS = false, class Mono>
+BN_DEVM void miller_loop_keyed_fold(Fp12& f, const G1Affine& pa, bool key_inf, const int32_t* lines, const int32_t* folds, uint32_t key, const G1Affine& pb,
+                                    Mono mono) {
+  if constexpr (F_LDS) BN_ASSUME_LDS(&f);
+  fp12_set_one(f);
+  lines = bn_wave_uniform(lines); folds = bn_wave_uniform(folds);
+  mono.uniform();
+  typedef const int32_t (*LinePtr)[2][2][BN_LIMBS];
+  typedef const int32_t (*FoldPtr)[5][2][BN_LIMBS];
+  const bool skip_a = pa.inf || key_inf, skip_b = pb.inf;
+#if defined(__HIPCC__)
+  const bool any_skip = __builtin_amdgcn_ballot_w64(skip_a || skip_b) != 0;
+#else
+  const bool any_skip = skip_a || skip_b;
+#endif
+  g1_monomials_put(mono, 0, pa);
+  g1_monomials_put(mono, 1, pb);
+  const LinePtr tab = (LinePtr)(lines + (size_t)key * (BN_N_FIXED_LINES * 2 * 2 * BN_LIMBS));
+  const FoldPtr fold = (FoldPtr)(folds + (size_t)key * (BN_N_FOLD_ROWS * 5 * 2 * BN_LIMBS));
+  auto folded_a = [&](int r) { LineProduct L; folded_row_product<286>(L, fold[r], pa, mono, 0, skip_a, any_skip); fp12_mul_line2(f, f, L.b0, L.b10, L.b11); };
+  auto folded_b = [&](int r) { LineProduct L; folded_row_product<287>(L, C_NEG_G2_FOLD[r], pb, mono, 1, skip_b, any_skip); fp12_mul_line2(f, f, L.b0, L.b10, L.b11); };
+  int idx = 0, r = 0;
+  for (int d = 0; d < 64; ++d) {
+    BN_SET_STEP_PRIORITY(d);
+    fp12_sqr(f, f);
+    const bool digit = C_ATE_NAF[d] != 0;
+    if (digit) folded_b(r);
+    if (!digit) {
+      KeyLine la;
+      la.c0 = fp2_load_const(tab[idx][0]); la.c1 = fp2_load_const(tab[idx][1]);
+      mul_by_two_table_lines(f, la, pa.x, pa.y, skip_a, idx, pb.x, pb.y, skip_b, any_skip);
+      ++idx;
+    } else { folded_a(r); ++r; idx += 2; }
+  }
+  folded_b(r);
+  folded_a(r);
+}
+#endif
 BN_DEV void mul_by_two_key_lines(Fp12& f, const KeyLine& la, const Fp& pax, const Fp& pay, bool skip_a, const KeyLine& lb, const Fp& pbx, const Fp& pby,
                                  bool skip_b, bool any_skip) {
   const Fp2 l0 = fp2_mul_fp(la.c0, pay), l1 = fp2_mul_fp(la.c1, pax);
diff --git a/bn254_amd/csrc/bn254_ws.h b/bn254_amd/csrc/bn254_ws.h
--- a/bn254_amd/csrc/bn254_ws.h
+++ b/bn254_amd/csrc/bn254_ws.h
@@ -173,6 +173,10 @@
 __attribute__((visibility("hidden"))) int bn254_lm_miller_verify_keyed(size_t n, Ws ws, const uint32_t* key_idx, KeyTable kt, hipStream_t s);
 __attribute__((visibility("hidden"))) int bn254_pair_miller_verify_keyed(size_t n, Ws ws, const uint32_t* key_idx, KeyTable kt, hipStream_t s, size_t base = 0,
                                                                          const uint32_t* map = nullptr, const uint32_t* count = nullptr);
+#define BN_KEY_FOLD_WORDS (5 * 2 * BN_LIMBS)
+__attribute__((visibility("hidden"))) int bn254_pair_miller_verify_keyed_fold(size_t n, Ws ws, const uint32_t* key_idx, KeyTable kt, const int32_t* fold,
+                                                                              hipStream_t s, size_t base = 0, const uint32_t* map = nullptr,
+                                                                              const uint32_t* count = nullptr);
 #define AGGD_KEYED_W1_MAX_SLOTS 65536
 __attribute__((visibility("hidden"))) int bn254_pair_aggd_keyed(size_t n_slots, int width, Ws ws, AggdSlots sl, const uint32_t* key_idx, KeyTable kt,
                                                                 size_t gbase, size_t pbase, uint32_t* pseg, int last, hipStream_t s);
@@ -220,6 +224,7 @@
 
 #define KEY_DEDUP_MAX_KEYS_DEFAULT 1024
 #define KEY_DEDUP_MIN_MULT_DEFAULT 16
+#define KEY_DEDUP_FOLD_DEFAULT 1
 #define KEY_DEDUP_MAX_KEYS_LIMIT 16384
 #define KD_MAX_PROBES 64u
 #define KD_EMPTY 0xFFFFFFFFu
@@ -235,6 +240,7 @@
   uint32_t* ctl;
   int32_t* lines;
   int32_t* c2;
+  int32_t* fold;
   uint8_t* st;
   uint8_t* inf;
   uint32_t* row_of;
@@ -248,7 +254,9 @@
 __attribute__((visibility("hidden"))) int bn254_kd_enqueue(const uint8_t* d_pks, size_t n, uint32_t flags, KeyDedup kd, int force_generic, int cache_reset,
                                                            int cache_on, hipStream_t s);
 #define KD_BYTES_PER_ITEM ((size_t)(2 * 4 + 2) * sizeof(uint32_t))
-#define KD_BYTES_PER_KEY ((size_t)BN_N_FIXED_LINES * (BN_KEY_LINE_WORDS + 2 * BN_LIMBS) * sizeof(int32_t) + (4 + 32 + 4) * sizeof(uint32_t) + 2)
+#define KD_FOLD_KEY_WORDS (BN_N_FOLD_ROWS * BN_KEY_FOLD_WORDS)
+static_assert(KD_FOLD_KEY_WORDS >= BN_N_FIXED_LINES * 2 * BN_LIMBS, "a key's raw c2 fits where its folded rows go");
+#define KD_BYTES_PER_KEY ((size_t)(BN_N_FIXED_LINES * BN_KEY_LINE_WORDS + KD_FOLD_KEY_WORDS) * sizeof(int32_t) + (4 + 32 + 4) * sizeof(uint32_t) + 2)
 
 __attribute__((visibility("hidden"))) int bn254_trio_miller_verify(size_t n, Ws ws, hipStream_t s, int mode = 0);
 __attribute__((visibility("hidden"))) int bn254_quad_miller_verify(size_t n, Ws ws, hipStream_t s, int mode = 0);
diff --git a/bn254_amd/csrc/gen_constants.py b/bn254_amd/csrc/gen_constants.py
--- a/bn254_amd/csrc/gen_constants.py
+++ b/bn254_amd/csrc/gen_constants.py
@@ -436,6 +436,24 @@
     for ln in lines:
         o.append("  {%s, %s, %s}," % (c_fp2(ln[0]), c_fp2(ln[1]), c_fp2(ln[2])))
     o.append("};")
+    fold_first = []
+    idx = 0
+    for d in naf:
+        if d:
+            fold_first.append(idx)
+        idx += 2 if d else 1
+    fold_first.append(idx)
+    assert idx + 2 == len(lines)
+    o.append("#define BN_N_FOLD_ROWS %d" % len(fold_first))
+    o.append("BN_CONST unsigned char C_FOLD_FIRST[BN_N_FOLD_ROWS] = {%s};  /* folded row -> its first table line (the second one follows it); the last row = the two closing lines */" %
+             ", ".join(str(i) for i in fold_first))
+    o.append("/* the folded rows (K0 .. K4) of Q = -G2::one() */")
+    o.append("BN_CONST int32_t C_NEG_G2_FOLD[BN_N_FOLD_ROWS][5][2][BN_LIMBS] = {")
+    for i in fold_first:
+        (a0, a1, _), (b0, b1, _) = lines[i], lines[i + 1]
+        ks = (mul(a0, b0), add(mul(a0, b1), mul(a1, b0)), mul(a1, b1), add(a0, b0), add(a1, b1))
+        o.append("  {%s}," % ", ".join(c_fp2(k) for k in ks))
+    o.append("};")
     o.append("")
     path = os.path.join(here, "bn254_constants.h")
     with open(path, "w") as f:
diff --git a/bn254_amd/engine.py b/bn254_amd/engine.py
--- a/bn254_amd/engine.py
+++ b/bn254_amd/engine.py
@@ -42,6 +42,7 @@
 OPT_BITMAP_RAND_MIN_TUPLES = 33
 OPT_BITMAP_RAND_GROUP_TUPLES = 34
 OPT_BITMAP_RAND_MAX_KEYS = 35
+OPT_KEY_DEDUP_FOLD = 44
 OPT_KEY_CACHE = 36
 OPT_COLLECT_RAND_MIN_SHARES = 38
 OPT_COLLECT_RAND_MIN_PER_KEY = 39
@@ -150,6 +151,11 @@
         st, inf = ctypes.create_string_buffer(max(count, 1)), ctypes.create_string_buffer(max(count, 1))
         _check("bn254_debug_key_tables", self._lib.bn254_debug_key_tables(self._h, which, first, count, words, rep, st, inf))
         return list(words), (list(rep)[:count] if which == 0 else None), st.raw[:count], inf.raw[:count]
+
+    def debug_key_fold_tables(self, first, count):
+        words = (ctypes.c_int32 * (count * 22 * 90))()
+        _check("bn254_debug_key_fold_tables", self._lib.bn254_debug_key_fold_tables(self._h, first, count, words))
+        return list(words)
 
     def debug_agg_tables_info(self):
         o = (ctypes.c_uint64 * 5)()
diff --git a/include/bn254_hip.h b/include/bn254_hip.h
--- a/include/bn254_hip.h
+++ b/include/bn254_hip.h
@@ -282,6 +282,7 @@
 #define BN254_OPT_HASH_MAX_TRIES 2
 #define BN254_OPT_G2_FIXED_BASE 19
 #define BN254_OPT_KEY_DEDUP_FORCE_GENERIC 23
+#define BN254_OPT_KEY_DEDUP_FOLD 44
 #define BN254_OPT_KEY_DEDUP_HASH_BITS 24
 #define BN254_OPT_AGGD_KEYED_ROUTE 25
 #define BN254_OPT_AGG_RAND_GROUP_PAIRS 27
@@ -293,6 +294,7 @@
 int bn254_debug_key_dedup_last(bn254_ctx *ctx, uint32_t out[5]);
 int bn254_debug_key_cache_last(bn254_ctx *ctx, uint32_t out[5]);
 int bn254_debug_key_tables(bn254_ctx *ctx, int which, size_t first, size_t count, int32_t *lines, uint32_t *rep, uint8_t *st, uint8_t *inf);
+int bn254_debug_key_fold_tables(bn254_ctx *ctx, size_t first, size_t count, int32_t *rows);
 int bn254_debug_agg_tables(bn254_ctx *ctx, int which, size_t first, size_t count, uint8_t *points, uint8_t *flags);
 int bn254_debug_agg_rand_last(bn254_ctx *ctx, uint64_t out[6]);
 int bn254_debug_agg_rand_sums(bn254_ctx *ctx, uint64_t dims[2], size_t group_cap, size_t pair_cap, uint32_t *nagg, uint8_t *verdict,
```

New measurement: 16.04 million, median of 6. +1.1%, better.
